# jantonguirao/nvImageCodec

Measured on AMD Instinct MI355X. Metric: images/sec, batched 1920x1080 4:2:0 baseline JPEG decode to interleaved RGB u8, higher is better.
Workload: dtype int32

## Files before the change

### include/hipjpeg.h

```cpp
#ifndef HIPJPEG_H_
#define HIPJPEG_H_

#include <stddef.h>
#include <stdint.h>

#ifdef __cplusplus
extern "C" {
#endif

#define HIPJPEG_API __attribute__((visibility("default")))

typedef enum {
    HIPJPEG_STATUS_SUCCESS = 0,
    HIPJPEG_STATUS_INVALID_ARGUMENT = 1,
    HIPJPEG_STATUS_BAD_JPEG = 2,
    HIPJPEG_STATUS_UNSUPPORTED = 3,
    HIPJPEG_STATUS_TRUNCATED = 4,
    HIPJPEG_STATUS_CORRUPT = 5,
    HIPJPEG_STATUS_ALLOC_FAILED = 6,
    HIPJPEG_STATUS_HIP_ERROR = 7,
    HIPJPEG_STATUS_NO_DEVICE = 8,
    HIPJPEG_STATUS_BUFFER_TOO_SMALL = 9,
    HIPJPEG_STATUS_INTERNAL_ERROR = 10
} hipjpegStatus_t;

typedef enum {
    HIPJPEG_OUTPUT_RGBI = 0,
    HIPJPEG_OUTPUT_BGRI = 1,
    HIPJPEG_OUTPUT_RGB_PLANAR = 2,
    HIPJPEG_OUTPUT_BGR_PLANAR = 3,
    HIPJPEG_OUTPUT_Y = 4,
    HIPJPEG_OUTPUT_YUV_PLANAR = 5
} hipjpegOutputFormat_t;

typedef enum {
    HIPJPEG_CSS_444 = 0,
    HIPJPEG_CSS_422 = 1,
    HIPJPEG_CSS_420 = 2,
    HIPJPEG_CSS_440 = 3,
    HIPJPEG_CSS_411 = 4,
    HIPJPEG_CSS_410 = 5,
    HIPJPEG_CSS_GRAY = 6,
    HIPJPEG_CSS_410V = 7,
    HIPJPEG_CSS_UNKNOWN = -1
} hipjpegChromaSubsampling_t;

#define HIPJPEG_FLAG_FANCY_UPSAMPLING 1u
#define HIPJPEG_FLAG_GPU_HUFFMAN 2u
#define HIPJPEG_FLAG_FAST_IDCT 4u
#define HIPJPEG_FLAG_GPU_PROGRESSIVE_INTERVALS 16u

typedef struct {
    int32_t width, height, num_components;
    int32_t sof_marker;
    int32_t color_model;
    int32_t subsampling;
    int32_t restart_interval, num_scans;
    int32_t h[4], v[4];
    int32_t blocks_w[4], blocks_h[4];
    int32_t samp_w[4], samp_h[4];
    uint64_t coef_bytes;
} hipjpegImageInfo_t;

typedef struct {
    void* plane[3];
    uint32_t pitch[3];
} hipjpegOutput_t;

typedef struct {
    int32_t x0, y0, x1, y1;
    int32_t orientation;
} hipjpegTransform_t;

typedef struct hipjpegHandle* hipjpegHandle_t;

HIPJPEG_API const char* hipjpegStatusString(hipjpegStatus_t status);
HIPJPEG_API int hipjpegVersion(void);
HIPJPEG_API hipjpegStatus_t hipjpegTestSetFault(const char* site, int countdown);
HIPJPEG_API int hipjpegTestDoubleReports(void);
HIPJPEG_API int32_t hipjpegTestHostFallbacks(hipjpegHandle_t handle);
HIPJPEG_API hipjpegStatus_t hipjpegTestKernelFlavours(hipjpegHandle_t handle, int32_t plane_units[1], int32_t luma_units[3]);
HIPJPEG_API int32_t hipjpegTestFusedUnits(hipjpegHandle_t handle);

HIPJPEG_API int32_t hipjpegTestScanChunkDrops(const uint8_t* data, size_t length, int scan_index, uint32_t* drops, int32_t capacity);
HIPJPEG_API int32_t hipjpegTestPairSteps(const uint8_t bits[16], const uint8_t* vals, int32_t nvals, uint32_t* steps);

HIPJPEG_API hipjpegStatus_t hipjpegTestSetScratchFill(int byte);

HIPJPEG_API hipjpegStatus_t hipjpegGetImageInfo(const uint8_t* data, size_t length, hipjpegImageInfo_t* info);

HIPJPEG_API hipjpegStatus_t hipjpegEntropyDecodeHost(const uint8_t* data, size_t length, int16_t* coef, size_t coef_capacity_bytes,
                                                     uint64_t comp_offsets[4], uint16_t qtables[256]);

HIPJPEG_API hipjpegStatus_t hipjpegEntropyDecodeHostSparse(const uint8_t* data, size_t length, uint8_t* stream, size_t capacity_bytes, size_t* stream_bytes,
                                                           uint64_t table_offsets[4]);

HIPJPEG_API hipjpegStatus_t hipjpegEntropyDecodeGpuAlgorithmHost(const uint8_t* data, size_t length, int16_t* coef,
                                                                 size_t coef_capacity_bytes, uint64_t comp_offsets[4],
                                                                 int32_t* sync_passes);

HIPJPEG_API hipjpegStatus_t hipjpegEntropyDecodeGpuIntervalAlgorithmHost(const uint8_t* data, size_t length, int16_t* coef,
                                                                         size_t coef_capacity_bytes, uint64_t comp_offsets[4]);

HIPJPEG_API hipjpegStatus_t hipjpegCreate(hipjpegHandle_t* handle, int device_id, int num_host_threads);
HIPJPEG_API hipjpegStatus_t hipjpegDestroy(hipjpegHandle_t handle);

typedef struct {
    int (*device_malloc)(void* ctx, void** ptr, size_t size, void* stream);
    int (*device_free)(void* ctx, void* ptr, size_t size, void* stream);
    void* device_ctx;
    int (*pinned_malloc)(void* ctx, void** ptr, size_t size, void* stream);
    int (*pinned_free)(void* ctx, void* ptr, size_t size, void* stream);
    void* pinned_ctx;
} hipjpegAllocators_t;
HIPJPEG_API hipjpegStatus_t hipjpegSetAllocators(hipjpegHandle_t handle, const hipjpegAllocators_t* allocators);

HIPJPEG_API hipjpegStatus_t hipjpegDecodeBatch(hipjpegHandle_t handle, const uint8_t* const* data, const size_t* lengths, int batch_size,
                                               const hipjpegOutput_t* outputs, hipjpegOutputFormat_t format, unsigned flags,
                                               hipjpegStatus_t* statuses, void* stream);

HIPJPEG_API hipjpegStatus_t hipjpegDecodeBatchSetTransforms(hipjpegHandle_t handle, const hipjpegTransform_t* transforms, int batch_size);

HIPJPEG_API hipjpegStatus_t hipjpegGetScaledImageSize(int32_t width, int32_t height, int32_t scale_denom, int32_t* scaled_width,
                                                      int32_t* scaled_height);
HIPJPEG_API hipjpegStatus_t hipjpegDecodeBatchSetScales(hipjpegHandle_t handle, const int32_t* scale_denoms, int batch_size);

HIPJPEG_API hipjpegStatus_t hipjpegDecodeBatchHost(hipjpegHandle_t handle, const uint8_t* const* data, const size_t* lengths, int batch_size,
                                                   const hipjpegOutput_t* outputs, hipjpegOutputFormat_t format, unsigned flags,
                                                   hipjpegStatus_t* statuses);
HIPJPEG_API hipjpegStatus_t hipjpegDecodeBatchTransfer(hipjpegHandle_t handle, void* stream);
HIPJPEG_API hipjpegStatus_t hipjpegDecodeBatchDevice(hipjpegHandle_t handle, void* stream);
HIPJPEG_API hipjpegStatus_t hipjpegDecodeBatchDeviceKernel(hipjpegHandle_t handle, int which, void* stream);
HIPJPEG_API hipjpegStatus_t hipjpegDecodeBatchSubmit(hipjpegHandle_t handle, const uint8_t* const* data, const size_t* lengths, int batch_size,
                                                     const hipjpegOutput_t* outputs, hipjpegOutputFormat_t format, unsigned flags, void* stream);
HIPJPEG_API hipjpegStatus_t hipjpegDecodeBatchWait(hipjpegHandle_t handle, hipjpegStatus_t* statuses, int batch_size);
HIPJPEG_API int32_t hipjpegDecodeBatchZeroCopyImages(hipjpegHandle_t handle);
HIPJPEG_API int32_t hipjpegDecodeBatchIntervalImages(hipjpegHandle_t handle);
HIPJPEG_API int32_t hipjpegDecodeBatchIntervalTakeovers(hipjpegHandle_t handle);
HIPJPEG_API hipjpegStatus_t hipjpegDecodeBatchTransferStats(hipjpegHandle_t handle, uint64_t* h2d_bytes, int32_t* sparse_images);

HIPJPEG_API hipjpegStatus_t hipjpegSetHybridHuffmanThreshold(hipjpegHandle_t handle, uint64_t pixels);

HIPJPEG_API hipjpegStatus_t hipjpegSetPipelineDepth(hipjpegHandle_t handle, int depth);
HIPJPEG_API hipjpegStatus_t hipjpegDecodeBatchGetStatuses(hipjpegHandle_t handle, hipjpegStatus_t* statuses, int batch_size);
HIPJPEG_API hipjpegStatus_t hipjpegDecodeBatchEntropyStats(hipjpegHandle_t handle, int32_t* gpu_images, int32_t* sync_launches,
                                                           uint64_t* stream_bytes);
HIPJPEG_API hipjpegStatus_t hipjpegDecodeBatchStats(hipjpegHandle_t handle, int32_t num_units[3], uint64_t* coef_bytes,
                                                    uint64_t* output_bytes);

typedef struct {
    const void* plane[3];
    uint32_t pitch[3];
    int32_t width, height;
} hipjpegEncodeInput_t;

typedef struct {
    int32_t quality;
    int32_t subsampling;
    int32_t input_format;
    int32_t restart_interval;
    int32_t optimized_huffman;
    int32_t progressive;
} hipjpegEncodeParams_t;
#define HIPJPEG_FLAG_GPU_RESTART_INTERVALS 8u
#define HIPJPEG_FLAG_GPU_PROGRESSIVE_RESTART 32u

HIPJPEG_API hipjpegStatus_t hipjpegEncodeBatchDevice(hipjpegHandle_t handle, const hipjpegEncodeInput_t* inputs,
                                                     const hipjpegEncodeParams_t* params, int batch_size, hipjpegStatus_t* statuses, void* stream);
// ... 134 lines not shown
```

### nvimagecodec_amd/csrc/decoder_core.cpp

```cpp
#include "decoder_core.h"
#include "host_copy.h"

#include <hip/hip_runtime_api.h>

#include <algorithm>
#include <cstdio>
#include <cstdlib>
#include <cstring>
#include <numeric>

#include "coefficients_core.h"
#include "decode_kernels.h"
#include "diagnostics.h"
#include "entropy_decode.h"
#include "gpu_huffman_host.h"
#include "progressive_gpu_host.h"
#include "transcode_core.h"

namespace hipjpeg {

namespace {
int out_planes(OutFormat fmt) { return (fmt == kOutInterleavedRGB || fmt == kOutInterleavedBGR || fmt == kOutY) ? 1 : 3; }
int out_bpp(OutFormat fmt) { return (fmt == kOutInterleavedRGB || fmt == kOutInterleavedBGR) ? 3 : 1; }

// ... 197 lines not shown
                                  hipjpegOutputFormat_t format, unsigned flags, hipjpegStatus_t* statuses,
                                  const hipjpegOutputFormat_t* formats, ForkJoinPool* pool, const hipjpegTransform_t* transforms,
                                  const int32_t* scale_denoms)
{
    pool_ = pool;
    coef_only_ = false;
    tensor_source_ = false;
    PlanArgs a{data, lengths, outputs, format, flags, formats, transforms, nullptr};
    a.scales = scale_denoms;
    return plan_attempts(a, n, statuses);
}

hipjpegStatus_t DecodeBatch::plan_tensors(const hipjpegCoefficientInfo_t* infos, const hipjpegCoefficientPlanes_t* planes, int n,
                                          const hipjpegOutput_t* outputs, hipjpegOutputFormat_t format, unsigned flags, hipjpegStatus_t* statuses,
                                          ForkJoinPool* pool, const hipjpegTransform_t* transforms)
{
    if (n > 0 && (!infos || !planes)) return HIPJPEG_STATUS_INVALID_ARGUMENT;
    pool_ = pool;
    coef_only_ = false;
    tensor_source_ = true;
    tensor_planes_ = planes;
    PlanArgs a{nullptr, nullptr, outputs, format, flags & ~HIPJPEG_FLAG_GPU_HUFFMAN, nullptr, transforms, nullptr};
    a.infos = infos;
    a.tensors = planes;
    return plan_attempts(a, n, statuses);
}

hipjpegStatus_t DecodeBatch::plan_coefficients(const uint8_t* const* data, const size_t* lengths, int n, unsigned flags, hipjpegStatus_t* statuses,
                                               ForkJoinPool* pool, const hipjpegTranscodeParams_t* params, bool any_frame)
{
    pool_ = pool;
    coef_only_ = true;
    tensor_source_ = false;
    return plan_attempts(PlanArgs{data, lengths, nullptr, HIPJPEG_OUTPUT_RGBI, flags & (HIPJPEG_FLAG_GPU_HUFFMAN | HIPJPEG_FLAG_GPU_PROGRESSIVE_INTERVALS), nullptr, nullptr, nullptr, params, any_frame}, n,
                         statuses);
}

hipjpegStatus_t DecodeBatch::plan_attempts(const PlanArgs& a, int n, hipjpegStatus_t* statuses)
{
    std::vector<char> give_up((size_t)std::max(n, 0), 0);
    PlanArgs args = a;
    args.give_up = give_up.data();
    for (int attempt = 0;; attempt++) {
        const hipjpegStatus_t st = plan_once(args, n, statuses);
        if (st != HIPJPEG_STATUS_ALLOC_FAILED || attempt >= 16) return st;
        int worst = -1;
        size_t worst_bytes = 0;
        for (int i = 0; i < n; i++) {
            if (images_[i].status != HIPJPEG_STATUS_SUCCESS) continue;
            const size_t b = images_[i].frame.total_blocks() * 128 + (size_t)images_[i].frame.width * images_[i].frame.height;
            if (b >= worst_bytes) {
                worst_bytes = b;
                worst = i;
            }
        }
        if (worst < 0) return st;
        give_up[worst] = 1;
    }
}

hipjpegStatus_t DecodeBatch::plan_once(const PlanArgs& a, int n, hipjpegStatus_t* statuses)
{
    if (n < 0 || (n > 0 && (((!a.data || !a.lengths) && !a.infos) || (!a.outputs && !coef_only_)))) return HIPJPEG_STATUS_INVALID_ARGUMENT;
    if ((int)a.format < 0 || (int)a.format > (int)HIPJPEG_OUTPUT_YUV_PLANAR) return HIPJPEG_STATUS_INVALID_ARGUMENT;
    ScopedRange range("hipjpeg plan (parse headers, lay out staging)");
    fault_point("plan");
    finalized_ = false;
    host_drops_missing_.store(false, std::memory_order_relaxed);
    images_.resize((size_t)n);
    desc_.resize((size_t)n);
    fast_idct_ = (a.flags & HIPJPEG_FLAG_FAST_IDCT) != 0;
    entropy_done_ = false;
    entropy_pending_ = false;
    huff_images_.clear();
    huff_to_image_.clear();
    seq_gpu_images_ = 0;
    prog_images_.clear();
    prog_to_image_.clear();
    prog_walk_images_ = 0;
    interval_takeover_images_ = 0;
    host_fallback_images_ = 0;
    xform_desc_.clear();
    prog_slot_words_ = 0;
    max_huff_units_ = max_pool_words_ = 0;
    coef_bytes_ = output_bytes_ = 0;
    if (pool_ && n > 1)
        pool_->parallel_for(n, [&](int i, int) { prepare(i, a); });
    else
        for (int i = 0; i < n; i++) prepare(i, a);
    demote_progressive_lds();
    for (int tail = 0; tail < 2; tail++) {
        for (int i = 0; i < n; i++) {
            PlannedImage& im = images_[i];
            if (im.status != HIPJPEG_STATUS_SUCCESS || !im.gpu_prog || (int)im.gpu_prog_intervals != tail) continue;
            im.prog_index = (int)prog_to_image_.size();
            prog_to_image_.push_back(i);
        }
        if (tail == 0) prog_walk_images_ = prog_to_image_.size();
    }
    Sizing s(n);
    for (int i = 0; i < n; i++) size_image(i, s);
    layout(s);
    const hipjpegStatus_t st = reserve(s);
    if (st != HIPJPEG_STATUS_SUCCESS) return st;
    bind_pointers(s);
    h2d_used_ = staging_.h2d_bytes;
    if (statuses)
        for (int i = 0; i < n; i++) statuses[i] = images_[i].status;
    return HIPJPEG_STATUS_SUCCESS;
}

void DecodeBatch::prepare(int i, const PlanArgs& a)
{
    PlannedImage& im = images_[i];
    im = PlannedImage();
    desc_[i] = DecodeImage();
    im.data = a.infos ? nullptr : a.data[i];
    im.size = a.infos ? 0 : a.lengths[i];
    if (a.formats && ((int)a.formats[i] < 0 || (int)a.formats[i] > (int)HIPJPEG_OUTPUT_YUV_PLANAR)) {
        im.status = HIPJPEG_STATUS_INVALID_ARGUMENT;
        return;
    }
    const OutFormat fmt = (OutFormat)(a.formats ? a.formats[i] : a.format);
    bool fancy = (a.flags & HIPJPEG_FLAG_FANCY_UPSAMPLING) != 0;
    const FrameInfo& f = im.frame;
    const int denom = a.scales ? a.scales[i] : 1;
    if (denom != 1 && denom != 2 && denom != 4 && denom != 8) {
        im.status = HIPJPEG_STATUS_INVALID_ARGUMENT;
        return;
    }
    im.scale_k = 8 / denom;
    if (a.infos)
        im.status = coefficient_frame(a.infos[i], a.tensors[i], &im.frame);
    else
        im.status = a.data[i] ? status_from_parse(parse_jpeg(a.data[i], a.lengths[i], &im.frame)) : HIPJPEG_STATUS_INVALID_ARGUMENT;
    if (im.status == HIPJPEG_STATUS_SUCCESS && ((uint64_t)f.width * (uint64_t)f.height * (uint64_t)f.ncomp >= max_image_samples() || a.give_up[i]))
        im.status = HIPJPEG_STATUS_ALLOC_FAILED;
    if (coef_only_) {
        TranscodePicture pic;
        im.variant = -4;
        const bool grayscale = a.transcode && (a.transcode[i].orientation & HIPJPEG_TRANSCODE_GRAYSCALE) != 0;
        if (im.status == HIPJPEG_STATUS_SUCCESS && !a.any_frame) im.status = transcode_picture(f, grayscale, &pic);
    } else {
        im.pic_w = f.width;
        im.pic_h = f.height;
        if (im.status == HIPJPEG_STATUS_SUCCESS && im.scale_k != 8) {
            im.variant = -5;
            im.pic_w = scaled_extent(f.width, im.scale_k);
            im.pic_h = scaled_extent(f.height, im.scale_k);
            fancy = fancy && im.scale_k > 1;
            if (!choose_scaled(f, fmt, im.scale_k, im.scaled_size)) im.status = HIPJPEG_STATUS_UNSUPPORTED;
        } else if (im.status == HIPJPEG_STATUS_SUCCESS && !choose_variant(f, fmt, fancy, &im.variant))
            im.status = HIPJPEG_STATUS_UNSUPPORTED;
        for (int p = 0; im.status == HIPJPEG_STATUS_SUCCESS && p < (fmt == kOutPlanarYUV ? f.ncomp : out_planes(fmt)); p++)
            if (!a.outputs[i].plane[p]) im.status = HIPJPEG_STATUS_INVALID_ARGUMENT;
        if (im.status == HIPJPEG_STATUS_SUCCESS && a.transforms) im.status = normalise_transform(im, a.transforms[i], fmt);
        if (im.status == HIPJPEG_STATUS_SUCCESS && !pitch_ok(i, a.outputs[i], fmt)) im.status = HIPJPEG_STATUS_INVALID_ARGUMENT;
    }
    const bool want_gpu_entropy = (a.flags & HIPJPEG_FLAG_GPU_HUFFMAN) != 0;
    const bool big_enough = (uint64_t)f.width * (uint64_t)f.height > gpu_entropy_min_pixels_ || gpu_entropy_min_pixels_ == 0;
    if (im.status == HIPJPEG_STATUS_SUCCESS && want_gpu_entropy && big_enough && gpu_entropy_eligible(f)) {
        im.gpu_entropy = true;
        for (const ScanHeader& sc : f.scans) im.pool_words = std::max(im.pool_words, gpu_pool_words(sc));
        im.fused_layout = f.scans.size() == 1;
        for (int c = 0; c < f.scans[0].ncomp; c++) im.fused_layout = im.fused_layout && f.scans[0].comp_index[c] == c;
        static const bool zero_copy = getenv("HIPJPEG_NO_ZERO_COPY") == nullptr;
        if (zero_copy) {
// ... 126 lines not shown
    }
    for (int c = 0; c < f.ncomp && im.variant == -5; c++) {
        const Component& k = f.comp[c];
        DecodeComponent& dc = d.comp[c];
        const size_t sz = (size_t)im.scaled_size[c];
        dc.plane_pitch = (uint32_t)align_up((size_t)k.blocks_w * sz + 16, 16);
        s.plane_off[(size_t)i * 4 + c] = s.planes.take(align_up((size_t)dc.plane_pitch * k.blocks_h * sz + 16, 256));
        s.units += ((size_t)k.blocks_w * k.blocks_h + kBlocksPerUnit - 1) / kBlocksPerUnit;
    }
    if (im.variant == -5) s.units += ((size_t)im.pic_h + kScaledRowsPerUnit - 1) / kScaledRowsPerUnit;
    for (int c = 0; c < f.ncomp && im.variant != -5; c++) {
        const Component& k = f.comp[c];
        const Route route = component_route(im.variant, fmt, c);
        if (route == kRoutePlane) {
            DecodeComponent& dc = d.comp[c];
            dc.plane_pitch = (uint32_t)align_up((size_t)k.blocks_w * 8 + 16, 16);
            s.plane_off[(size_t)i * 4 + c] = s.planes.take(align_up((size_t)dc.plane_pitch * k.blocks_h * 8 + 16, 256));
        }
        if (route != kRouteNone) s.units += ((size_t)k.blocks_w * k.blocks_h + kBlocksPerUnit - 1) / kBlocksPerUnit;
        if (c == 0 && im.variant >= 0) s.units += (size_t)((k.blocks_w + kLumaTileW - 1) / kLumaTileW) * (size_t)((k.blocks_h + kLumaTileH - 1) / kLumaTileH);
    }
    if (im.variant == -1 || im.variant == -3) s.units += (size_t)f.height;
    coef_bytes_ += f.total_blocks() * 128;
    if (tensor_source_)
        for (int c = 0; c < f.ncomp; c++) s.tensor_units += ((size_t)f.comp[c].blocks_w * f.comp[c].blocks_h + kRelayoutBlocksPerUnit - 1) / kRelayoutBlocksPerUnit;
    if (fmt == kOutPlanarYUV)
        for (int c = 0; c < f.ncomp; c++) output_bytes_ += (uint64_t)f.comp[c].samp_w * f.comp[c].samp_h;
    else
        output_bytes_ += (uint64_t)im.pic_w * im.pic_h * (fmt == kOutY ? 1 : 3);
    if (!im.gpu_entropy) return;
    if (im.gpu_prog) im.tables_offset = s.pools.take(align_up(im.pool_words * 2, 64), 1);
    if (!im.gpu_prog)
        for (size_t sidx = 0; sidx < f.scans.size(); sidx++) {
            const ScanHeader& sc = f.scans[sidx];
            const size_t blocks = (size_t)scan_mcus_x(f, sc) * scan_mcus_y(f, sc) * scan_blocks_per_mcu(f, sc);
            im.seq[sidx].dc_diff_offset = s.blocks.take(((blocks + 31) & ~(size_t)31) * 2, 1);
        }
    for (int c = 0; c < f.ncomp; c++) {
        const size_t nblk = (size_t)f.comp[c].blocks_w * f.comp[c].blocks_h;
        im.dc_plane_offset[c] = s.blocks.take(((nblk + 31) & ~(size_t)31) * 2, 1);
        if (im.gpu_prog) s.prog_units += (nblk + 255) / 256;
    }
    if (im.gpu_prog) {
        im.prog_huff_first = (uint32_t)s.prog_scans;
        s.prog_scans += f.scans.size();
        for (size_t sidx = 0; sidx < f.scans.size(); sidx++) {
            const ScanHeader& sc = f.scans[sidx];
            s.scan(sc, &im.prog_raw_offset[sidx], &im.prog_stream_offset[sidx], &im.prog_first_chunk[sidx]);
            if (sc.ss != 0) {
                const int cc = sc.comp_index[0];
                const size_t nb = (size_t)((f.comp[cc].samp_w + 7) / 8) * (size_t)((f.comp[cc].samp_h + 7) / 8);
                im.prog_pos_offset[sidx] = s.prog_pos.take(((nb + 63) & ~(size_t)63) * 4, 1);
                prog_slot_words_ = std::max<unsigned>(prog_slot_words_, (unsigned)prog_table_words(sc.ac[sc.ta[0]]));
            } else if (sc.ah == 0) {
                for (int k = 0; k < sc.ncomp; k++)
                    prog_slot_words_ = std::max<unsigned>(prog_slot_words_, (unsigned)prog_table_words(sc.dc[sc.td[k]]));
            }
        }
        if (im.gpu_prog_intervals) {
            int ac_scans[4] = {0, 0, 0, 0};
            for (size_t sidx = 0; sidx < f.scans.size(); sidx++) {
                const ScanHeader& sc = f.scans[sidx];
                const size_t count = sc.rst_after.size() + 1;
                im.prog_start_offset[sidx] = s.boundaries.take(align_up(sc.rst_after.size() * 4, 64), 1);
                if (sc.ss == 0 || ac_scans[sc.comp_index[0]]++ == 0) s.prog_iv_units += (count + kProgIntervalLanes - 1) / kProgIntervalLanes;
            }
            for (int c = 0; c < f.ncomp; c++)
                if (ac_scans[c] > 1)
                    im.prog_hist_offset[c] = s.prog_pos.take((size_t)((f.comp[c].samp_w + 7) / 8) * (size_t)((f.comp[c].samp_h + 7) / 8) * 8, 8);
        }
        return;
    }
    static_assert(sizeof(im.seq) / sizeof(im.seq[0]) == (size_t)kMaxSeqScans, "one SeqScan per scan gpu_entropy_eligible() admits");
    im.huff_index = (int)huff_to_image_.size();
    im.huff_count = (int)f.scans.size();
    seq_gpu_images_++;
    for (size_t sidx = 0; sidx < f.scans.size(); sidx++) {
        const ScanHeader& sc = f.scans[sidx];
        PlannedImage::SeqScan& q = im.seq[sidx];
        huff_to_image_.push_back(i);
        const size_t nsub = (s.scan(sc, &q.raw_offset, &q.stream_offset, &q.first_chunk) * 8 + kSubseqBits - 1) / kSubseqBits;
        const size_t mcus = (size_t)scan_mcus_x(f, sc) * scan_mcus_y(f, sc);
        s.subseq += nsub;
        max_huff_units_ += std::max<size_t>((nsub + kHuffOwn - 1) / kHuffOwn, 1);
        q.pool_words = gpu_pool_words(sc);
        q.tables_offset = s.pools.take(align_up(q.pool_words * 2, 64), 1);
        max_pool_words_ = std::max(max_pool_words_, q.pool_words);
        s.huff_wunits += (mcus + kHuffMcusPerWg - 1) / kHuffMcusPerWg + 1;
        q.num_boundaries = (uint32_t)sc.rst_after.size();
        q.boundary_offset = s.boundaries.take(sc.restart_interval ? align_up(((size_t)q.num_boundaries + nsub + 1) * 4, 64) : 0, 1);
        q.block_pos_offset = s.block_pos.take(((mcus * scan_blocks_per_mcu(f, sc) + 63) & ~(size_t)63) * 4, 1);
    }
}

void DecodeBatch::layout(const Sizing& s)
{
    const size_t ng = huff_to_image_.size(), chunks = s.chunks.end;
    StagingLayout& L = staging_;
    Carve c;
    L.desc = c.take(sizeof(DecodeImage) * images_.size());
    L.units = c.take(sizeof(WorkUnit) * s.units);
    L.huff_desc = c.take(sizeof(HuffImage) * (ng + s.prog_scans));
    L.huff_units = c.take(sizeof(HuffUnit) * max_huff_units_);
    L.huff_wunits = c.take(sizeof(HuffUnit) * s.huff_wunits);
    L.huff_dc_units = c.take(sizeof(HuffUnit) * ng * 4);
    L.huff_chunk_units = c.take(sizeof(HuffUnit) * chunks);
    L.huff_drops = c.take(sizeof(uint32_t) * chunks);
    L.xform_desc = c.take(sizeof(TransformImage) * xform_desc_.size());
    L.xform_units = c.take(sizeof(WorkUnit) * s.xform_units);
    L.prog_desc = c.take(sizeof(ProgImage) * prog_to_image_.size());
    L.prog_units = c.take(sizeof(HuffUnit) * s.prog_units);
    L.prog_iv_desc = c.take(sizeof(ProgIntervalImage) * (prog_to_image_.size() - prog_walk_images_));
    L.prog_iv_units = c.take(sizeof(HuffUnit) * s.prog_iv_units);
    L.tensor_planes = c.take(tensor_source_ ? sizeof(CoefPlane) * 4 * images_.size() : 0);
    L.tensor_units = c.take(sizeof(RelayoutUnit) * s.tensor_units);
    L.tables = c.take(s.pools.end);
    L.boundaries = c.take(s.boundaries.end);
    L.streams = c.take(s.raw.end);
    L.coef = c.take(0);
    static const bool sparse_enabled = getenv("HIPJPEG_DENSE_STAGING") == nullptr;
    sparse_mode_ = sparse_enabled && !coef_only_ && !tensor_source_;
    host_coef_used_.store(0);
    for (int pass = 0; pass < 2; pass++) {
        if (pass == 1) {
            L.h2d_bytes = c.end;
            L.gpu_coef_begin = c.take(0);
        }
        for (PlannedImage& im : images_) {
            if (im.status != HIPJPEG_STATUS_SUCCESS || (int)(im.gpu_entropy || tensor_source_) != pass) continue;
            if (pass == 0 && sparse_mode_) c.end += 256;
            for (int k = 0; k < im.frame.ncomp; k++) im.coef_offset[k] = c.take((size_t)im.frame.comp[k].blocks_w * im.frame.comp[k].blocks_h * 128, 1);
            if (!im.gpu_entropy) continue;
            if (im.gpu_prog) {
                im.tables_offset += L.tables;
                for (size_t sidx = 0; sidx < im.frame.scans.size(); sidx++) im.prog_raw_offset[sidx] += L.streams;
                for (size_t sidx = 0; sidx < im.frame.scans.size() && im.gpu_prog_intervals; sidx++) im.prog_start_offset[sidx] += L.boundaries;
            } else {
                for (int sidx = 0; sidx < im.huff_count; sidx++) {
                    im.seq[sidx].raw_offset += L.streams;
                    im.seq[sidx].boundary_offset += L.boundaries;
                    im.seq[sidx].tables_offset += L.tables;
                }
            }
        }
    }
    L.total = c.end;
    total_subseq_ = s.subseq;
    Carve w;
    w.take(total_subseq_ * 8);
    scratch_.first_block = w.take(total_subseq_ * 4);
    scratch_.changed = w.take(256);
    scratch_.incoming = w.take(max_huff_units_ * 8);
    scratch_.tail = w.take(max_huff_units_ * (kTailTaskBytes + 4));
    scratch_.dc_diff = w.take(s.blocks.end);
    scratch_.block_pos = w.take(s.block_pos.end);
    scratch_.records = w.take(total_subseq_ * kRecShorts * 2);
    scratch_.walkers = w.take(max_huff_units_ * 4);
    scratch_.verdicts = w.take(verdict_bytes());
    scratch_.drops = w.take(chunks * 4);
    scratch_.prog_pos = w.take(s.prog_pos.end);
    scratch_.group_sums = w.take(s.huff_wunits * 16);
    scratch_.streams = w.take(s.streams.end);
    scratch_.total = w.end;
}

hipjpegStatus_t DecodeBatch::reserve(const Sizing& s)
{
    if (hipSetDevice(device_id_) != hipSuccess) return HIPJPEG_STATUS_NO_DEVICE;
    if (in_flight_) {
        if (hipEventSynchronize((hipEvent_t)done_event_) != hipSuccess) return HIPJPEG_STATUS_HIP_ERROR;
        in_flight_ = false;
    }
    hipjpegStatus_t st;
    if ((st = pinned_.reserve(staging_.h2d_bytes + 256 + verdict_bytes())) != HIPJPEG_STATUS_SUCCESS) return st;
    if ((st = device_.reserve(staging_.total + 256)) != HIPJPEG_STATUS_SUCCESS) return st;
    if ((st = planes_.reserve(s.planes.end + 256)) != HIPJPEG_STATUS_SUCCESS) return st;
    if (!huff_to_image_.empty() || s.prog_scans) return work_.reserve(scratch_.total + 256);
    return HIPJPEG_STATUS_SUCCESS;
}

void DecodeBatch::bind_pointers(const Sizing& s)
{
    huff_images_.assign(huff_to_image_.size() + s.prog_scans, HuffImage());
    prog_images_.assign(prog_to_image_.size(), ProgImage());
    prog_iv_images_.assign(prog_to_image_.size() - prog_walk_images_, ProgIntervalImage());
    size_t k = 0;
// ... 157 lines not shown
    build_entropy_units();
    build_tensor_units();
    h2d_used_ = sparse_mode_ ? std::min(staging_.h2d_bytes, align_up(staging_.coef + host_coef_used_.load(), 256)) : staging_.h2d_bytes;
    stage_tables();
    finalized_ = true;
}

void DecodeBatch::build_pixel_units()
{
    for (UnitList* l : {&plane_units_, &fused_plane_units_, &generic_units_, &cmyk_units_, &xform_units_, &reduced_units_, &scaled_color_units_}) l->units.clear();
    for (auto* lists : {&luma_units_, &fused_luma_units_})
        for (auto& row : *lists)
            for (UnitList& l : row) l.units.clear();
    for (size_t i = 0; i < images_.size(); i++) {
        const PlannedImage& im = images_[i];
        if (im.status != HIPJPEG_STATUS_SUCCESS) continue;
        const FrameInfo& f = im.frame;
        DecodeImage& d = desc_[i];
        if (sparse_mode_ && !im.gpu_entropy) {
            size_t blocks_before = 0;
            for (int c = 0; c < f.ncomp; c++) {
                DecodeComponent& dc = d.comp[c];
                if (im.sparse) {
                    dc.coef = at<const int16_t>(device_, im.host_coef_offset);
                    dc.block_off = at<const uint32_t>(device_, im.host_coef_offset) + blocks_before;
                    blocks_before += (size_t)f.comp[c].blocks_w * f.comp[c].blocks_h;
                } else {
                    dc.coef = at<const int16_t>(device_, im.coef_offset[c]);
                    dc.block_off = nullptr;
                }
                dc.dc = dc.coef;
                dc.dc_stride = 64;
            }
        }
        const OutFormat fmt = (OutFormat)d.out_format;
        const bool fused = fused_ && im.gpu_entropy && !im.gpu_prog;
        d.huff_index = fused ? (uint32_t)im.huff_index : 0u;
        for (int c = 0; c < f.ncomp && im.variant == -5; c++) {
            const uint32_t nblk = (uint32_t)f.comp[c].blocks_w * f.comp[c].blocks_h;
            std::vector<WorkUnit>& list = (im.scaled_size[c] == 8 ? plane_units_ : reduced_units_).units;
            for (uint32_t b = 0; b < nblk; b += kBlocksPerUnit) list.push_back(WorkUnit{(uint32_t)i, b, (uint32_t)c, (uint32_t)kToPlane});
        }
        for (int y = 0; y < im.pic_h && im.variant == -5; y += kScaledRowsPerUnit) scaled_color_units_.units.push_back(WorkUnit{(uint32_t)i, (uint32_t)y, 0u, 0u});
        for (int c = 0; c < f.ncomp && im.variant != -5; c++) {
            const Route route = component_route(im.variant, fmt, c);
            if (route == kRouteNone) continue;
            const uint32_t nblk = (uint32_t)f.comp[c].blocks_w * f.comp[c].blocks_h;
            const uint32_t mode = route == kRouteOutput ? (uint32_t)(kToOutput | (c << 8)) : (uint32_t)kToPlane;
            for (uint32_t b = 0; b < nblk; b += kBlocksPerUnit) (fused ? fused_plane_units_ : plane_units_).units.push_back(WorkUnit{(uint32_t)i, b, (uint32_t)c, mode});
        }
        if (im.variant >= 0) {
            uint32_t real_rows = (uint32_t)(f.height + 7) / 8, first_row = 0, first_col = 0, end_col = (uint32_t)f.comp[0].blocks_w;
            if (im.has_transform) {
                first_row = (uint32_t)im.transform.y0 / 8 / kLumaTileH * kLumaTileH;
                real_rows = std::min(real_rows, (uint32_t)(im.transform.y1 + 7) / 8);
                first_col = (uint32_t)im.transform.x0 / 8 / kLumaTileW * kLumaTileW;
                end_col = std::min(end_col, (uint32_t)(im.transform.x1 + 7) / 8);
            }
            const bool everyday = im.variant != kVarGray && d.color_model == 1 && (d.flags & kFlagFancyUpsampling) &&
                                  (im.variant == kVar11 || im.variant == kVar12 || d.comp[1].samp_w > 2);
            const int layout = !everyday ? 0 : (fmt == kOutInterleavedRGB || fmt == kOutInterleavedBGR) ? 1 : (fmt == kOutPlanarRGB || fmt == kOutPlanarBGR) ? 2 : 0;
            std::vector<WorkUnit>& tiles = (fused ? fused_luma_units_ : luma_units_)[layout][im.variant].units;
            const uint32_t span = end_col - first_col, ragged = span % kLumaTileW;
            const uint32_t wide_end = (ragged != 0 && ragged <= kLumaTileW / 2) ? end_col - ragged : end_col;
            for (uint32_t by = first_row; by < real_rows; by += kLumaTileH)
                for (uint32_t bx = first_col; bx < wide_end; bx += kLumaTileW) tiles.push_back(WorkUnit{(uint32_t)i, bx, by, 0u});
            if (wide_end < end_col)
                for (uint32_t by = first_row; by < real_rows; by += 2 * kLumaTileH) tiles.push_back(WorkUnit{(uint32_t)i, wide_end, by, 1u});
        } else if (im.variant == -1) {
            for (int y = 0; y < f.height; y++) generic_units_.units.push_back(WorkUnit{(uint32_t)i, (uint32_t)y, 0u, 0u});
        } else if (im.variant == -3) {
            for (int y = 0; y < f.height; y++) cmyk_units_.units.push_back(WorkUnit{(uint32_t)i, (uint32_t)y, 0u, 0u});
        }
        if (im.has_transform) {
            const TransformImage& t = xform_desc_[im.xform_index];
            for (int oy = 0; oy < t.out_h; oy += kTransformRowsPerUnit) xform_units_.units.push_back(WorkUnit{(uint32_t)im.xform_index, (uint32_t)oy, 0u, 0u});
        }
    }
}

void DecodeBatch::build_entropy_units()
{
    for (std::vector<HuffUnit>* v : {&huff_units_, &huff_wunits_, &huff_chunk_units_, &huff_dc_units_, &prog_units_}) v->clear();
    uint32_t first_subseq = 0;
    stream_bytes_total_ = 0;
    huff_zero_.clear();
    for (size_t g = 0; g < huff_to_image_.size(); g++) {
        const PlannedImage& im = images_[huff_to_image_[g]];
        HuffImage& h = huff_images_[g];
        if (im.status != HIPJPEG_STATUS_SUCCESS) {
            h.num_subseq = 0;
            continue;
        }
        const int sidx = (int)g - im.huff_index;
        const ScanHeader& sc = im.frame.scans[sidx];
        const PlannedImage::SeqScan& q = im.seq[sidx];
        h.stream = work_.data() + scratch_.streams + q.stream_offset;
        h.raw = device_.data() + q.raw_offset;
        h.raw_src = im.input_pinned ? im.input_device_view + sc.data_begin : nullptr;
        if (h.restart_interval) {
            h.boundaries = at<const uint32_t>(device_, q.boundary_offset);
            h.sub_boundary = h.boundaries + h.num_boundaries;
        }
        h.raw_bytes = q.stream_bytes;
        h.first_chunk = q.first_chunk;
        for (uint32_t c = 0; c * (uint32_t)kDestuffChunk < q.stream_bytes; c++) huff_chunk_units_.push_back(HuffUnit{(uint32_t)g, c});
        h.pool = at<const uint16_t>(device_, q.tables_offset);
        h.dc_diff = at<int16_t>(work_, scratch_.dc_diff + q.dc_diff_offset);
        h.block_pos = at<uint32_t>(work_, scratch_.block_pos + q.block_pos_offset);
        for (uint32_t m = 0; m < h.mcus_x * h.mcus_y; m += kHuffMcusPerWg) huff_wunits_.push_back(HuffUnit{(uint32_t)g, m});
        for (int i = 0; i < sc.ncomp; i++) {
            const int c = sc.comp_index[i];
            const Component& fc = im.frame.comp[c];
            h.coef[i] = at<int16_t>(device_, im.coef_offset[c]);
            h.dc_plane[i] = at<int16_t>(work_, scratch_.dc_diff + im.dc_plane_offset[c]);
            const size_t bw = (size_t)fc.blocks_w, bh = (size_t)fc.blocks_h;
            if (sc.ncomp == 1 && (h.mcus_x < bw || h.mcus_y < bh)) {
                const size_t first = h.mcus_x < bw ? 0 : (size_t)h.mcus_y * bw, n = bw * bh - first;
                huff_zero_.push_back(ZeroFill{reinterpret_cast<uint8_t*>(h.coef[i] + first * 64), n * 128, 1, 0});
                huff_zero_.push_back(ZeroFill{reinterpret_cast<uint8_t*>(h.dc_plane[i] + first), n * 2, 1, 0});
            }
        }
        h.first_subseq = first_subseq;
        first_subseq += h.num_subseq;
        for (uint32_t j = 0; j == 0 || j < h.num_subseq; j += kHuffOwn) huff_units_.push_back(HuffUnit{(uint32_t)g, j});
        if (h.restart_interval)
            for (uint32_t i = 0; i < h.ncomp; i++) huff_dc_units_.push_back(HuffUnit{(uint32_t)g, i});
        stream_bytes_total_ += q.stream_bytes;
    }
    merge_zero_fills();
    total_subseq_ = first_subseq;
    for (size_t q = 0; q < prog_images_.size(); q++) {
        const PlannedImage& im = images_[prog_to_image_[q]];
        ProgImage& pi = prog_images_[q];
        if (im.status != HIPJPEG_STATUS_SUCCESS) {
            pi.num_scans = 0;
            pi.ncomp = 0;
            pi.dc_len = 0;
            memset(pi.chain_len, 0, sizeof pi.chain_len);
            continue;
        }
        const FrameInfo& f = im.frame;
        for (size_t sidx = 0; sidx < f.scans.size(); sidx++) {
            const size_t hidx = huff_to_image_.size() + im.prog_huff_first + sidx;
            HuffImage& h = huff_images_[hidx];
            h.stream = work_.data() + scratch_.streams + im.prog_stream_offset[sidx];
            h.raw = device_.data() + im.prog_raw_offset[sidx];
            ProgScan& ps = pi.scan[sidx];
            ps.stream = h.stream;
            ps.huff_image = (uint32_t)hidx;
            ps.block_pos = f.scans[sidx].ss != 0 ? at<uint32_t>(work_, scratch_.prog_pos + im.prog_pos_offset[sidx]) : nullptr;
            for (uint32_t c = 0; c * (uint32_t)kDestuffChunk < h.raw_bytes; c++) huff_chunk_units_.push_back(HuffUnit{(uint32_t)hidx, c});
        }
        pi.pool = at<const uint16_t>(device_, im.tables_offset);
        for (int c = 0; c < f.ncomp; c++) {
            pi.coef[c] = at<int16_t>(device_, im.coef_offset[c]);
            pi.dc_plane[c] = at<int16_t>(work_, scratch_.dc_diff + im.dc_plane_offset[c]);
            const uint32_t nblk = (uint32_t)f.comp[c].blocks_w * f.comp[c].blocks_h;
            for (uint32_t b = 0; b < nblk; b += 256) prog_units_.push_back(HuffUnit{(uint32_t)q, ((uint32_t)c << 28) | b});
        }
        stream_bytes_total_ += im.stream_bytes;
    }
    prog_iv_units_.clear();
    prog_iv_dc_first_.clear();
    uint32_t dc_scans = 0;
    for (size_t q = prog_walk_images_; q < prog_images_.size(); q++) {
        const PlannedImage& im = images_[prog_to_image_[q]];
        if (im.status != HIPJPEG_STATUS_SUCCESS) continue;
        const uint32_t rel = (uint32_t)(q - prog_walk_images_);
        ProgIntervalImage& iv = prog_iv_images_[rel];
        for (size_t sidx = 0; sidx < im.frame.scans.size(); sidx++) iv.scan[sidx].first_start = (uint32_t)((im.prog_start_offset[sidx] - staging_.boundaries) / 4);
        for (int c = 0; c < im.frame.ncomp; c++) {
            iv.hist[c] = prog_images_[q].chain_len[c] > 1 ? at<unsigned long long>(work_, scratch_.prog_pos + im.prog_hist_offset[c]) : nullptr;
            for (uint32_t first = 0; prog_images_[q].chain_len[c] > 0 && first < iv.ac_count[c]; first += kProgIntervalLanes)
                prog_iv_units_.push_back(HuffUnit{rel, ((uint32_t)c << 28) | first});
        }
        dc_scans = std::max(dc_scans, prog_images_[q].dc_len);
    }
    for (uint32_t d = 0; d < dc_scans; d++) {
        prog_iv_dc_first_.push_back(prog_iv_units_.size());
        for (size_t q = prog_walk_images_; q < prog_images_.size(); q++) {
            const ProgImage& pi = prog_images_[q];
            if (pi.dc_len <= d) continue;
            const uint32_t count = prog_iv_images_[q - prog_walk_images_].scan[pi.dc_chain[d]].count;
            for (uint32_t first = 0; first < count; first += kProgIntervalLanes) prog_iv_units_.push_back(HuffUnit{(uint32_t)(q - prog_walk_images_), first});
        }
    }
    prog_iv_dc_first_.push_back(prog_iv_units_.size());
}

void DecodeBatch::merge_zero_fills()
{
    std::vector<ZeroFill> in, out;
    in.swap(huff_zero_);
    for (int series = 0; series < 2; series++) {
        for (size_t a = (size_t)series; a < in.size();) {
            ZeroFill z = in[a];
            size_t b = a + 2;
            if (b < in.size() && in[b].bytes == z.bytes && in[b].ptr > z.ptr && (size_t)(in[b].ptr - z.ptr) >= z.bytes) {
                z.pitch = (size_t)(in[b].ptr - z.ptr);
                while (b < in.size() && in[b].bytes == z.bytes && in[b].ptr == z.ptr + z.count * z.pitch) {
                    z.count++;
                    b += 2;
                }
            }
            out.push_back(z);
            a += 2 * z.count;
        }
    }
    huff_zero_.swap(out);
}

static void deal_rows_to_xcds(std::vector<WorkUnit>& v)
{
    if (v.size() < 64) return;
    constexpr size_t kXcds = 8;
    std::vector<WorkUnit> queue[kXcds], rest, out;
    out.reserve(v.size());
    auto flush = [&]() {
        size_t taken[kXcds] = {0};
        for (bool any = true; any;) {
            any = false;
            for (size_t q = 0; q < kXcds; q++)
                if (taken[q] < queue[q].size()) {
                    out.push_back(queue[q][taken[q]++]);
                    any = true;
                }
        }
        out.insert(out.end(), rest.begin(), rest.end());
        for (auto& q : queue) q.clear();
        rest.clear();
    };
    size_t row = 0;
    for (size_t a = 0; a < v.size();) {
        size_t b = a + 1;
        while (b < v.size() && v[b].image == v[a].image && v[b].comp == v[a].comp && v[b].mode == v[a].mode) b++;
        if (a > 0 && v[a].image != v[a - 1].image) {
            flush();
            row = 0;
        }
        if (v[a].mode != 0) {
            rest.insert(rest.end(), v.begin() + (long)a, v.begin() + (long)b);
        } else {
            std::vector<WorkUnit>& q = queue[row++ % kXcds];
            q.insert(q.end(), v.begin() + (long)a, v.begin() + (long)b);
        }
        a = b;
    }
    flush();
    v.swap(out);
}

void DecodeBatch::stage_tables()
{
    auto stage = [&](UnitList& list, Carve& where) {
        list.offset = where.take(list.units.size() * sizeof(WorkUnit), 1);
        copy_table(pinned_, list.offset, list.units);
    };
    copy_table(pinned_, staging_.desc, desc_);
    Carve units{staging_.units};
    stage(plane_units_, units);
    for (auto& lists : luma_units_)
        for (UnitList& l : lists) {
            deal_rows_to_xcds(l.units);
            stage(l, units);
        }
    stage(fused_plane_units_, units);
    for (auto& lists : fused_luma_units_)
        for (UnitList& l : lists) stage(l, units);
    stage(generic_units_, units);
    stage(cmyk_units_, units);
    stage(reduced_units_, units);
    stage(scaled_color_units_, units);
    Carve xform{staging_.xform_units};
    stage(xform_units_, xform);
    copy_table(pinned_, staging_.xform_desc, xform_desc_);
    copy_table(pinned_, staging_.tensor_planes, tensor_table_);
    copy_table(pinned_, staging_.tensor_units, tensor_units_);
    copy_table(pinned_, staging_.prog_desc, prog_images_);
    copy_table(pinned_, staging_.prog_units, prog_units_);
    copy_table(pinned_, staging_.prog_iv_desc, prog_iv_images_);
    copy_table(pinned_, staging_.prog_iv_units, prog_iv_units_);
    copy_table(pinned_, staging_.huff_desc, huff_images_);
    copy_table(pinned_, staging_.huff_units, huff_units_);
    copy_table(pinned_, staging_.huff_wunits, huff_wunits_);
    copy_table(pinned_, staging_.huff_dc_units, huff_dc_units_);
    copy_table(pinned_, staging_.huff_chunk_units, huff_chunk_units_);
}

hipjpegStatus_t DecodeBatch::transfer(void* stream, bool kernels_on_other_stream)
{
    if (!finalized_) return HIPJPEG_STATUS_INVALID_ARGUMENT;
    ScopedRange range("hipjpeg transfer to device");
    fault_point("transfer");
    entropy_done_ = false;
    pixels_launched_ = false;
    if (h2d_used_ == 0) return HIPJPEG_STATUS_SUCCESS;
    zero_copy_images_ = 0;
    for (const PlannedImage& im : images_) zero_copy_images_ += (im.status == HIPJPEG_STATUS_SUCCESS && im.gpu_entropy && !im.gpu_prog && im.input_pinned) ? 1 : 0;
    hipError_t e = hipSuccess;
    if (zero_copy_images_ == 0) {
        e = hipMemcpyAsync(device_.data(), pinned_.data(), h2d_used_, hipMemcpyHostToDevice, (hipStream_t)stream);
    } else {
        hipStream_t s = (hipStream_t)stream;
        const size_t rb = std::min(staging_.streams, h2d_used_), re = std::min(staging_.coef, h2d_used_);
        if (rb > 0) e = hipMemcpyAsync(device_.data(), pinned_.data(), rb, hipMemcpyHostToDevice, s);
        if (e == hipSuccess && re > rb) e = hipMemsetAsync(device_.data() + rb, 0x01, re - rb, s);
        if (e == hipSuccess && h2d_used_ > re) e = hipMemcpyAsync(device_.data() + re, pinned_.data() + re, h2d_used_ - re, hipMemcpyHostToDevice, s);
        for (const PlannedImage& im : images_) {
            if (e != hipSuccess) break;
            if (im.status != HIPJPEG_STATUS_SUCCESS || !im.gpu_entropy) continue;
            if (im.gpu_prog) {
                for (size_t sidx = 0; sidx < im.frame.scans.size() && e == hipSuccess; sidx++) {
                    const ScanHeader& sc = im.frame.scans[sidx];
                    const size_t len = sc.data_end - sc.data_begin;
                    if (len) e = hipMemcpyAsync(device_.data() + im.prog_raw_offset[sidx], pinned_.data() + im.prog_raw_offset[sidx], align_up(len, 16) + 16, hipMemcpyHostToDevice, s);
                }
                continue;
            }
            for (int sidx = 0; sidx < im.huff_count && e == hipSuccess && !im.input_pinned; sidx++) {
                const PlannedImage::SeqScan& q = im.seq[sidx];
                e = hipMemcpyAsync(device_.data() + q.raw_offset, pinned_.data() + q.raw_offset, align_up((size_t)q.stream_bytes, 16) + 16, hipMemcpyHostToDevice, s);
            }
        }
        if (e == hipSuccess && launch_gather_raw(at<const HuffImage>(device_, staging_.huff_desc), at<const HuffUnit>(device_, staging_.huff_chunk_units),
                                                 (int)huff_chunk_units_.size(), stream) != 0) e = hipErrorLaunchFailure;
    }
    if (e == hipSuccess && kernels_on_other_stream) {
        if (!ensure_event(&copied_event_)) return HIPJPEG_STATUS_HIP_ERROR;
        e = hipEventRecord((hipEvent_t)copied_event_, (hipStream_t)stream);
        copy_pending_ = true;
    }
    return e == hipSuccess ? HIPJPEG_STATUS_SUCCESS : HIPJPEG_STATUS_HIP_ERROR;
}

hipjpegStatus_t DecodeBatch::enqueue_gpu_entropy(void* stream)
{
    hipStream_t s = (hipStream_t)stream;
    entropy_done_ = true;
    if (huff_units_.empty() && prog_units_.empty()) return HIPJPEG_STATUS_SUCCESS;
    EntropyLaunch L = entropy_launch_args();
    if (huff_chunk_units_.empty() && hipMemsetAsync(L.changed, 0, 256, s) != hipSuccess) return HIPJPEG_STATUS_HIP_ERROR;
    for (const ZeroFill& z : huff_zero_)
        if ((z.count == 1 ? hipMemsetAsync(z.ptr, 0, z.bytes, s) : hipMemset2DAsync(z.ptr, z.pitch, 0, z.bytes, z.count, s)) != hipSuccess)
            return HIPJPEG_STATUS_HIP_ERROR;
    static const bool force_device_count = getenv("HIPJPEG_DEVICE_DESTUFF_COUNT") != nullptr;
    const bool device_count = force_device_count || host_drops_missing_.load(std::memory_order_relaxed);
    if (launch_destuff(L.dimg, at<const HuffUnit>(device_, staging_.huff_chunk_units), (int)huff_chunk_units_.size(),
                       device_count ? at<uint32_t>(work_, scratch_.drops) : at<uint32_t>(device_, staging_.huff_drops),
                       device_count, L.changed, stream) != 0)
        return HIPJPEG_STATUS_HIP_ERROR;
    if (!prog_units_.empty()) {
        const hipjpegStatus_t ps = enqueue_progressive(stream);
        if (ps != HIPJPEG_STATUS_SUCCESS) return ps;
    }
    if (huff_units_.empty()) {
        entropy_pending_ = true;
        return HIPJPEG_STATUS_SUCCESS;
    }
    static const int tail_after = getenv("HIPJPEG_TAIL_AFTER") ? atoi(getenv("HIPJPEG_TAIL_AFTER")) : 2;
    uint16_t* tail_tasks = at<uint16_t>(work_, scratch_.tail);
    uint32_t* tail_count = at<uint32_t>(work_, scratch_.tail + (size_t)max_huff_units_ * kTailTaskBytes);
    if (launch_huff_sync(L.dimg, L.dunits, L.nunits, L.states, L.incoming, L.changed, 1, tail_after > 0 ? tail_after : 1 << 20,
                         tail_after > 0 ? tail_tasks : nullptr, tail_after > 0 ? tail_count : nullptr, L.records, L.pool_bytes, stream) != 0)
        return HIPJPEG_STATUS_HIP_ERROR;
    if (launch_huff_sync(L.dimg, L.dunits, L.nunits, L.states, L.incoming, L.changed, 0, 1 << 20, nullptr, nullptr, L.records, L.pool_bytes, stream, 1) != 0)
        return HIPJPEG_STATUS_HIP_ERROR;
    if (!entropy_write_passes(L, stream)) return HIPJPEG_STATUS_HIP_ERROR;
    if (L.verdicts_out != L.host_changed && hipMemcpyAsync(L.host_changed, L.verdicts_out, verdict_bytes(), hipMemcpyDeviceToHost, s) != hipSuccess)
        return HIPJPEG_STATUS_HIP_ERROR;
    if (fused_ && hipMemcpyAsync(L.himg, L.dimg, sizeof(HuffImage) * huff_images_.size(), hipMemcpyDeviceToHost, s) != hipSuccess) return HIPJPEG_STATUS_HIP_ERROR;
    entropy_pending_ = true;
    return HIPJPEG_STATUS_SUCCESS;
}

hipjpegStatus_t DecodeBatch::enqueue_progressive(void* stream)
{
    ProgImage* dprog = at<ProgImage>(device_, staging_.prog_desc);
    const HuffImage* dimg = at<const HuffImage>(device_, staging_.huff_desc);
    const unsigned slot = (unsigned)align_up(std::max<unsigned>(prog_slot_words_, 256u), 64);
    unsigned dc_slots = 1, ac_waves = 0, rings = 0;
    for (size_t q = 0; q < prog_walk_images_; q++) {
        const ProgImage& pi = prog_images_[q];
        unsigned scans = 0, handovers = 0;
        for (int c = 0; c < 4; c++) {
            scans += pi.chain_len[c];
            handovers += pi.chain_len[c] > 0 ? pi.chain_len[c] - 1 : 0;
        }
        ac_waves = std::max(ac_waves, scans);
        rings = std::max(rings, handovers);
        for (uint32_t k = 0; k < pi.num_scans; k++)
            if (pi.scan[k].ss == 0 && pi.scan[k].ah == 0) dc_slots = std::max<unsigned>(dc_slots, pi.scan[k].ncomp);
    }
    static const bool debug_stats = getenv("HIPJPEG_DEBUG_TIMING") != nullptr;
    if (debug_stats)
        fprintf(stderr, "[hipjpeg] progressive walk: %zu images, %u + 1 waves per workgroup, %u table slots of %u entries, %u rings; interval kernels: %zu images\n",
                prog_walk_images_, ac_waves, dc_slots + ac_waves, slot, rings, prog_images_.size() - prog_walk_images_);
    if (launch_prog_walk(dprog, dimg, (int)prog_walk_images_, slot, dc_slots, ac_waves, rings, stream) != 0) return HIPJPEG_STATUS_HIP_ERROR;
    if (!prog_iv_units_.empty()) {
        ProgImage* tail = dprog + prog_walk_images_;
        const ProgIntervalImage* ivs = at<const ProgIntervalImage>(device_, staging_.prog_iv_desc);
        const uint32_t* starts = at<const uint32_t>(device_, staging_.boundaries);
        const HuffUnit* units = at<const HuffUnit>(device_, staging_.prog_iv_units);
        if (launch_prog_interval_ac(tail, ivs, dimg, starts, units, (int)prog_iv_dc_first_[0], slot, stream) != 0) return HIPJPEG_STATUS_HIP_ERROR;
        for (size_t d = 0; d + 1 < prog_iv_dc_first_.size(); d++)
            if (launch_prog_interval_dc(tail, ivs, dimg, starts, units + prog_iv_dc_first_[d], (int)(prog_iv_dc_first_[d + 1] - prog_iv_dc_first_[d]), (unsigned)d,
                                        slot, stream) != 0)
                return HIPJPEG_STATUS_HIP_ERROR;
    }
    if (launch_prog_replay(dprog, dimg, at<const HuffUnit>(device_, staging_.prog_units), (int)prog_units_.size(), slot, stream) != 0)
        return HIPJPEG_STATUS_HIP_ERROR;
    if (hipMemcpyAsync(pinned_.data() + staging_.prog_desc, dprog, sizeof(ProgImage) * prog_images_.size(), hipMemcpyDeviceToHost,
                       (hipStream_t)stream) != hipSuccess)
        return HIPJPEG_STATUS_HIP_ERROR;
    return HIPJPEG_STATUS_SUCCESS;
}

DecodeBatch::EntropyLaunch DecodeBatch::entropy_launch_args()
{
    EntropyLaunch L;
    L.dimg = at<HuffImage>(device_, staging_.huff_desc);
    L.dunits = at<const HuffUnit>(device_, staging_.huff_units);
    L.dwunits = at<const HuffUnit>(device_, staging_.huff_wunits);
    L.ddc = at<const HuffUnit>(device_, staging_.huff_dc_units);
    L.states = at<unsigned long long>(work_, 0);
    L.first_block = at<uint32_t>(work_, scratch_.first_block);
    static const bool full_position_pass = getenv("HIPJPEG_POSITION_PASS") != nullptr && atoi(getenv("HIPJPEG_POSITION_PASS")) != 0;
    L.records = at<uint16_t>(work_, scratch_.records);
    L.use_records = !full_position_pass && total_subseq_ * kRecShorts * 2 < (1ull << 32) ? L.records : nullptr;
    L.walkers = at<uint32_t>(work_, scratch_.walkers);
    L.group_sums = at<int32_t>(work_, scratch_.group_sums);
    L.changed = at<unsigned int>(work_, scratch_.changed);
    L.incoming = at<unsigned long long>(work_, scratch_.incoming);
    L.pool_bytes = (unsigned)align_up(max_pool_words_ * 2, 256);
    L.nunits = (int)huff_units_.size();
    L.host_changed = at<unsigned int>(pinned_, staging_.h2d_bytes);
    L.verdicts = L.host_changed + kHuffVerdictCounters;
    L.verdicts_out = pinned_.custom() ? at<unsigned int>(work_, scratch_.verdicts) : L.host_changed;
    L.himg = at<HuffImage>(pinned_, staging_.huff_desc);
    return L;
}

bool DecodeBatch::entropy_write_passes(const EntropyLaunch& L, void* stream)
{
    return launch_huff_write(L.dimg, L.dunits, L.nunits, L.dwunits, (int)huff_wunits_.size(), L.states, L.first_block, L.use_records, L.walkers, L.group_sums, L.pool_bytes,
                             stream, fused_) == 0 &&
           launch_huff_dc(L.dimg, L.ddc, (int)huff_dc_units_.size(), L.dwunits, (int)huff_wunits_.size(), L.group_sums, L.changed, L.verdicts_out, stream) == 0;
}

hipjpegStatus_t DecodeBatch::wait_done()
{
    if (!in_flight_) return HIPJPEG_STATUS_SUCCESS;
    return hipEventSynchronize((hipEvent_t)done_event_) == hipSuccess ? HIPJPEG_STATUS_SUCCESS : HIPJPEG_STATUS_HIP_ERROR;
}

hipjpegStatus_t DecodeBatch::resolve(void* stream)
{
    if (!entropy_pending_) return HIPJPEG_STATUS_SUCCESS;
    ScopedRange range("hipjpeg resolve (GPU entropy verdicts)");
    fault_point("resolve");
    hipStream_t s = (hipStream_t)stream;
    if (in_flight_ ? hipEventSynchronize((hipEvent_t)done_event_) != hipSuccess : hipStreamSynchronize(s) != hipSuccess) return HIPJPEG_STATUS_HIP_ERROR;
    entropy_pending_ = false;
    const EntropyLaunch L = entropy_launch_args();
    const size_t himg_bytes = sizeof(HuffImage) * huff_images_.size();
    bool redo_pixels = false;
    last_sync_launches_ = 2;
    static const bool debug_stats = getenv("HIPJPEG_DEBUG_TIMING") != nullptr;
    if (debug_stats)
        fprintf(stderr, "[hipjpeg] entropy: %d workgroups, launch 1 rounds avg %.2f max %u, tail rounds avg %.2f max %u; launch 2: %u rounds in total, max %u, %u boundary changes\n",
                L.nunits, (double)L.host_changed[2] / L.nunits, L.host_changed[3], (double)L.host_changed[6] / L.nunits, L.host_changed[7], L.host_changed[4],
                L.host_changed[5], L.host_changed[0]);
    bool converged = huff_units_.empty() || *L.host_changed == 0;
    constexpr int kExtraRippleLaunches = 4;
    uint32_t last_pass = 1;
    std::vector<char> unsettled(huff_images_.size(), 0);
    bool from_desc = fused_;
    if (!converged) {
        from_desc = true;
        for (int pass = 0; pass < kExtraRippleLaunches && !converged; pass++) {
            if (hipMemsetAsync(L.changed, 0, sizeof(unsigned int), s) != hipSuccess) return HIPJPEG_STATUS_HIP_ERROR;
            if (launch_huff_sync(L.dimg, L.dunits, L.nunits, L.states, L.incoming, L.changed, 0, 1 << 20, nullptr, nullptr, L.records, L.pool_bytes, stream, ++last_pass) != 0)
                return HIPJPEG_STATUS_HIP_ERROR;
            if (hipMemcpyAsync(L.host_changed, L.changed, sizeof(unsigned int), hipMemcpyDeviceToHost, s) != hipSuccess) return HIPJPEG_STATUS_HIP_ERROR;
            if (hipStreamSynchronize(s) != hipSuccess) return HIPJPEG_STATUS_HIP_ERROR;
            last_sync_launches_++;
            converged = *L.host_changed == 0;
        }
        if (hipMemcpyAsync(L.himg, L.dimg, himg_bytes, hipMemcpyDeviceToHost, s) != hipSuccess) return HIPJPEG_STATUS_HIP_ERROR;
        if (hipStreamSynchronize(s) != hipSuccess) return HIPJPEG_STATUS_HIP_ERROR;
        for (size_t g = 0; g < huff_to_image_.size(); g++) {
            unsettled[g] = L.himg[g].gave_up != 0 || (!converged && L.himg[g].moved_pass == last_pass);
            L.himg[g].status = 0;
        }
        if (hipMemcpyAsync(L.dimg, L.himg, himg_bytes, hipMemcpyHostToDevice, s) != hipSuccess) return HIPJPEG_STATUS_HIP_ERROR;
        if (!entropy_write_passes(L, stream)) return HIPJPEG_STATUS_HIP_ERROR;
        if (fused_ && pixels_launched_ && launch_pixel_kernels(stream, -1) != 0) return HIPJPEG_STATUS_HIP_ERROR;
        if (hipMemcpyAsync(L.himg, L.dimg, himg_bytes, hipMemcpyDeviceToHost, s) != hipSuccess) return HIPJPEG_STATUS_HIP_ERROR;
        if (hipStreamSynchronize(s) != hipSuccess) return HIPJPEG_STATUS_HIP_ERROR;
        redo_pixels = true;
    } else {
        for (size_t g = 0; g < huff_to_image_.size(); g++) unsettled[g] = from_desc ? L.himg[g].gave_up != 0 : huff_verdict_gave_up(L.verdicts[g]);
    }
    std::vector<int> takeover;
    for (size_t g = 0; g < huff_to_image_.size(); g++) {
        const int i = huff_to_image_[g];
        const bool flagged = from_desc ? L.himg[g].status != 0 : huff_verdict_status(L.verdicts[g]) != 0;
        if (images_[i].status == HIPJPEG_STATUS_SUCCESS && (flagged || unsettled[g]) && (takeover.empty() || takeover.back() != i))
            takeover.push_back(i);
    }
    host_fallback_images_ = (int)takeover.size();
    const ProgImage* hprog = at<const ProgImage>(pinned_, staging_.prog_desc);
    if (debug_stats && !prog_to_image_.empty()) print_progressive_timing(hprog);
    interval_takeover_images_ = 0;
    for (size_t q = 0; q < prog_to_image_.size(); q++)
        if (images_[prog_to_image_[q]].status == HIPJPEG_STATUS_SUCCESS && hprog[q].status != 0) {
            takeover.push_back(prog_to_image_[q]);
            interval_takeover_images_ += q >= prog_walk_images_ ? 1 : 0;
        }
    const hipjpegStatus_t st = take_over_on_host(takeover, &redo_pixels);
    if (st != HIPJPEG_STATUS_SUCCESS) return st;
    if (redo_pixels && pixels_launched_) {
        if (launch_pixel_kernels(stream, -1) != 0 || hipStreamSynchronize(s) != hipSuccess) return HIPJPEG_STATUS_HIP_ERROR;
    }
    return HIPJPEG_STATUS_SUCCESS;
}

void DecodeBatch::print_progressive_timing(const ProgImage* hprog) const
{
    const ProgImage& q0 = hprog[0];
    for (uint32_t k = 0; k < q0.num_scans; k++) {
        uint32_t lo = ~0u, hi = 0, cnt = 0;
        double sum = 0;
        for (size_t q = 0; q < prog_to_image_.size(); q++) {
            if (hprog[q].num_scans <= k) continue;
            const uint32_t t = hprog[q].scan[k].walk_ticks;
            lo = std::min(lo, t);
            hi = std::max(hi, t);
            sum += t;
            cnt++;
        }
        const uint32_t hw = q0.scan[k].pad_ticks[0];
        fprintf(stderr,
                "[hipjpeg] progressive image 0 scan %u (ss %u se %u ah %u al %u): walk %.3f ms, of which waiting for neighbours %.3f ms; se %u cu %u simd %u; "
                "all %u images: %.3f / %.3f / %.3f ms\n",
                k, q0.scan[k].ss, q0.scan[k].se, q0.scan[k].ah, q0.scan[k].al, q0.scan[k].walk_ticks * 1e-5, q0.scan[k].wait_ticks * 1e-5, (hw >> 13) & 7u,
                (hw >> 8) & 15u, (hw >> 4) & 3u, cnt, lo * 1e-5, cnt ? sum / cnt * 1e-5 : 0.0, hi * 1e-5);
    }
}

hipjpegStatus_t DecodeBatch::take_over_on_host(const std::vector<int>& takeover, bool* redo_pixels)
{
    constexpr size_t kHelping = 32;
    for (size_t first = 0; first < takeover.size(); first += kHelping) {
        const size_t count = std::min(kHelping, takeover.size() - first);
        std::vector<std::vector<int16_t>> coefs(count);
        std::vector<EntropyStatus> verdict(count, kEntropyOk);
        auto decode_one = [&](int j) {
            const PlannedImage& im = images_[takeover[first + j]];
            const FrameInfo& f = im.frame;
            coefs[j].assign(f.total_blocks() * 64, 0);
            int16_t* coef[4] = {nullptr, nullptr, nullptr, nullptr};
            size_t off = 0;
            for (int c = 0; c < f.ncomp; c++) {
                coef[c] = coefs[j].data() + off;
// ... 310 lines not shown
```

### nvimagecodec_amd/csrc/decoder_core.h

```cpp
#pragma once
#include <algorithm>
#include <atomic>
#include <cstddef>
#include <cstdint>
#include <vector>

#include "../../include/hipjpeg.h"
#include "coefficient_kernels.h"
#include "device_layout.h"
#include "decode_kernels.h"
#include "gpu_huffman.h"
#include "progressive_gpu.h"
#include "jpeg_syntax.h"
#include "staging.h"
#include "thread_pool.h"

namespace hipjpeg {

enum KernelVariant { kVarGray = 0, kVar11 = 1, kVar21 = 2, kVar22 = 3, kVar12 = 4, kNumLumaVariants = 5 };

struct UnitList {
    std::vector<WorkUnit> units;
    size_t offset = 0;
};
// ... 43 lines not shown
    uint32_t prog_first_chunk[kProgMaxScans] = {0};
    size_t prog_pos_offset[kProgMaxScans] = {0};
    bool gpu_prog_intervals = false;
    size_t prog_start_offset[kProgMaxScans] = {0};
    size_t prog_hist_offset[4] = {0, 0, 0, 0};
};

class DecodeBatch {
public:
    DecodeBatch(int device_id, const MemoryHooks* hooks);
    ~DecodeBatch();

    hipjpegStatus_t plan(const uint8_t* const* data, const size_t* lengths, int n, const hipjpegOutput_t* outputs,
                         hipjpegOutputFormat_t format, unsigned flags, hipjpegStatus_t* statuses,
                         const hipjpegOutputFormat_t* formats = nullptr, ForkJoinPool* pool = nullptr,
                         const hipjpegTransform_t* transforms = nullptr, const int32_t* scale_denoms = nullptr);
    hipjpegStatus_t plan_coefficients(const uint8_t* const* data, const size_t* lengths, int n, unsigned flags, hipjpegStatus_t* statuses,
                                      ForkJoinPool* pool, const hipjpegTranscodeParams_t* params = nullptr, bool any_frame = false);
    hipjpegStatus_t plan_tensors(const hipjpegCoefficientInfo_t* infos, const hipjpegCoefficientPlanes_t* planes, int n, const hipjpegOutput_t* outputs,
                                 hipjpegOutputFormat_t format, unsigned flags, hipjpegStatus_t* statuses, ForkJoinPool* pool,
                                 const hipjpegTransform_t* transforms = nullptr);
    hipjpegStatus_t import_tensors(void* stream);
    uint64_t imported_blocks() const { return imported_blocks_; }
    hipjpegStatus_t export_coefficients(const hipjpegCoefficientPlanes_t* planes, void* stream);
    uint64_t exported_blocks() const { return exported_blocks_; }
    const DecodeImage* device_descriptors() const { return at<const DecodeImage>(device_, staging_.desc); }
    void set_gpu_entropy_threshold(uint64_t pixels) { gpu_entropy_min_pixels_ = pixels; }
    void reject(int i, hipjpegStatus_t st)
    {
        if (i >= 0 && i < (int)images_.size() && images_[i].status == HIPJPEG_STATUS_SUCCESS) images_[i].status = st;
    }
    void output_size(int i, int* w, int* h) const;
    void entropy_stage(int i);
    void finalize(hipjpegStatus_t* statuses);
    hipjpegStatus_t transfer(void* stream, bool kernels_on_other_stream = false);
    hipjpegStatus_t launch(void* stream, int which = -1, void* entropy_stream = nullptr);
    hipjpegStatus_t resolve(void* stream);
    hipjpegStatus_t wait_done();
    void* last_stream() const { return last_stream_; }
    int gpu_entropy_images() const { return seq_gpu_images_ + (int)prog_to_image_.size(); }
    int last_sync_launches() const { return last_sync_launches_; }
    int host_fallback_images() const { return host_fallback_images_; }
    bool has_progressive() const { return !prog_to_image_.empty(); }
    int interval_images() const { return (int)(prog_to_image_.size() - prog_walk_images_); }
    int interval_takeover_images() const { return interval_takeover_images_; }
    uint64_t stream_bytes() const { return stream_bytes_total_; }
    int zero_copy_images() const { return zero_copy_images_; }
    uint64_t h2d_bytes() const { return h2d_used_; }
    int sparse_images() const { return (int)std::count_if(images_.begin(), images_.end(), [](const PlannedImage& im) { return im.sparse; }); }
    void flavour_units(int32_t* plane_units, int32_t luma_units[kNumLumaLayouts]) const { unit_counts(true, plane_units, luma_units); }
    int fused_units() const;

    int size() const { return (int)images_.size(); }
    const PlannedImage& image(int i) const { return images_[i]; }
    void stats(int32_t num_units[3], uint64_t* coef_bytes, uint64_t* output_bytes) const;

private:
    int device_id_;
    ForkJoinPool* pool_ = nullptr;
    uint64_t gpu_entropy_min_pixels_ = 0;

    struct PlanArgs;
    struct Sizing;
    hipjpegStatus_t plan_attempts(const PlanArgs& a, int n, hipjpegStatus_t* statuses);
    bool coef_only_ = false;
    bool tensor_source_ = false;
    const hipjpegCoefficientPlanes_t* tensor_planes_ = nullptr;
    std::vector<CoefPlane> tensor_table_;
    std::vector<RelayoutUnit> tensor_units_;
    void build_tensor_units();
    uint64_t imported_blocks_ = 0;
    hipjpegStatus_t plan_once(const PlanArgs& a, int n, hipjpegStatus_t* statuses);
    void prepare(int i, const PlanArgs& a);
    bool pitch_ok(int i, const hipjpegOutput_t& out, OutFormat fmt) const;
    void demote_progressive_lds();
    void size_image(int i, Sizing& s);
    void layout(const Sizing& s);
    hipjpegStatus_t reserve(const Sizing& s);
    void bind_pointers(const Sizing& s);
    Buffer pinned_, device_, planes_;
    Buffer export_pinned_, export_device_;
    uint64_t exported_blocks_ = 0;
    struct StagingLayout {
        size_t desc, units, huff_desc, huff_units, huff_wunits, huff_dc_units, huff_chunk_units, huff_drops, xform_desc, xform_units,
            prog_desc, prog_units, prog_iv_desc, prog_iv_units, tensor_planes, tensor_units, tables, boundaries, streams, coef, h2d_bytes, gpu_coef_begin, total;
    } staging_{};
    struct WorkLayout {
        size_t first_block, changed, incoming, tail, dc_diff, block_pos, records, walkers, verdicts, drops, prog_pos, group_sums, streams, total;
    } scratch_{};
    size_t verdict_bytes() const { return (kHuffVerdictCounters + huff_to_image_.size()) * sizeof(unsigned int); }
    Buffer work_;
    std::vector<PlannedImage> images_;
    std::vector<DecodeImage> desc_;
    bool fast_idct_ = false;
    uint64_t coef_bytes_ = 0, output_bytes_ = 0;
    bool sparse_mode_ = false;
    std::atomic<size_t> host_coef_used_{0};
    size_t h2d_used_ = 0;
    void stage_chunk_drops(const ScanHeader& sc, uint32_t first_chunk);
    void build_pixel_units();
    void build_entropy_units();
    void stage_tables();
    void merge_zero_fills();
    void unit_counts(bool plain, int32_t* plane, int32_t luma[kNumLumaLayouts]) const;
    UnitList plane_units_, luma_units_[kNumLumaLayouts][kNumLumaVariants], generic_units_, cmyk_units_, xform_units_;
    UnitList reduced_units_, scaled_color_units_;
    UnitList fused_plane_units_, fused_luma_units_[kNumLumaLayouts][kNumLumaVariants];
    bool fused_ = false;
    bool finalized_ = false;
    std::vector<TransformImage> xform_desc_;
    std::vector<HuffImage> huff_images_;
    std::vector<HuffUnit> huff_units_, huff_dc_units_;
    std::vector<int> huff_to_image_;
    int seq_gpu_images_ = 0;
    struct ZeroFill {
        uint8_t* ptr;
        size_t bytes, count, pitch;
    };
    std::vector<ZeroFill> huff_zero_;
    std::vector<HuffUnit> huff_wunits_;
    std::vector<HuffUnit> huff_chunk_units_;
    size_t total_subseq_ = 0, max_huff_units_ = 0, max_pool_words_ = 0;
    std::atomic<bool> host_drops_missing_{false};
    std::vector<ProgImage> prog_images_;
    std::vector<int> prog_to_image_;
    std::vector<HuffUnit> prog_units_;
    unsigned prog_slot_words_ = 0;
    size_t prog_walk_images_ = 0;
    std::vector<ProgIntervalImage> prog_iv_images_;
    std::vector<HuffUnit> prog_iv_units_;
    std::vector<size_t> prog_iv_dc_first_;
    uint64_t stream_bytes_total_ = 0;
    struct EntropyLaunch {
        HuffImage* dimg;
        const HuffUnit *dunits, *dwunits, *ddc;
        unsigned long long *states, *incoming;
        uint32_t* first_block;
        uint16_t* records;
        const uint16_t* use_records;
        uint32_t* walkers;
        int32_t* group_sums;
        unsigned int *changed, *host_changed;
        unsigned int* verdicts;
        unsigned int* verdicts_out;
        HuffImage* himg;
        unsigned pool_bytes;
        int nunits;
    };
    EntropyLaunch entropy_launch_args();
    bool entropy_write_passes(const EntropyLaunch& L, void* stream);
    hipjpegStatus_t enqueue_gpu_entropy(void* stream);
    hipjpegStatus_t enqueue_progressive(void* stream);
    int launch_pixel_kernels(void* stream, int which);
    int launch_taken_pixels(void* stream, int which);
    void print_progressive_timing(const ProgImage* hprog) const;
    hipjpegStatus_t take_over_on_host(const std::vector<int>& takeover, bool* redo_pixels);
    int zero_copy_images_ = 0;
    std::vector<int> host_taken_;
    void* taken_units_dev_ = nullptr;
    size_t taken_units_cap_ = 0;
    bool entropy_pending_ = false, pixels_launched_ = false, copy_pending_ = false, entropy_done_ = false;
    void* last_stream_ = nullptr;
    void* copied_event_ = nullptr;
    void* entropy_event_ = nullptr;
    void* done_event_ = nullptr;
    bool in_flight_ = false;
    int last_sync_launches_ = 0, host_fallback_images_ = 0, interval_takeover_images_ = 0;
};

hipjpegStatus_t status_from_parse(ParseStatus s);

}
```

### nvimagecodec_amd/csrc/gpu_huffman.h

```cpp
#pragma once
#include <cstdint>

#include "huffman_gpu_core.h"

namespace hipjpeg {

struct HuffUnit {
    uint32_t image;
    uint32_t first;
};

int launch_gather_raw(const HuffImage* images, const HuffUnit* chunk_units, int nchunks, void* stream);
int launch_destuff(HuffImage* images, const HuffUnit* chunk_units, int nchunks, uint32_t* drops, bool count_on_device, unsigned int* counters,
                   void* stream);

int launch_huff_sync(HuffImage* images, const HuffUnit* units, int nunits, unsigned long long* states, unsigned long long* incoming,
                     unsigned int* changed, int first_pass, int max_rounds, uint16_t* tail_tasks, uint32_t* tail_count, uint16_t* records,
                     unsigned pool_bytes, void* stream, unsigned pass_id = 0);
int launch_huff_write(HuffImage* images, const HuffUnit* sync_units, int nsync_units, const HuffUnit* block_units, int nblock_units,
                      const unsigned long long* states, uint32_t* first_block, const uint16_t* records, uint32_t* walkers,
                      int32_t* group_sums, unsigned pool_bytes, void* stream, bool dc_only = false);
constexpr int kHuffVerdictCounters = 8;
constexpr uint32_t huff_verdict(uint32_t status, uint32_t gave_up) { return (status & 0xFFu) | (gave_up ? 0x100u : 0u); }
constexpr uint32_t huff_verdict_status(uint32_t v) { return v & 0xFFu; }
constexpr bool huff_verdict_gave_up(uint32_t v) { return (v & 0x100u) != 0; }
int launch_huff_dc(const HuffImage* images, const HuffUnit* rst_units, int nrst_units, const HuffUnit* block_units, int nblock_units,
                   const int32_t* group_sums, const unsigned int* counters, unsigned int* verdicts, void* stream);

}
```

### nvimagecodec_amd/csrc/gpu_huffman.hip

```cpp
#include <hip/hip_runtime.h>

#include "gpu_huffman.h"
#include "huffman_gpu_core.h"
#include "kernel_common.h"

namespace hipjpeg {

namespace {

constexpr int kThreads = 256;

constexpr int kRowShift = kSubseqWords == 32 ? 5 : kSubseqWords == 16 ? 4 : kSubseqWords == 64 ? 6 : -1;
static_assert(kRowShift > 0, "subsequences of 512, 1024 or 2048 bits");

struct KSlot {
    int16_t* base;
    uint32_t stride_y, stride_x;
};

constexpr int kStagedExtra = 2;
constexpr int kRowWords = kSubseqWords + kStagedExtra;
static_assert(kSubseqWords % 4 == 0 && kStagedExtra == 2, "stage_rows: 16-byte groups and one 8-byte group per row");
__host__ __device__ constexpr int staged_lds_words(int rows) { return rows * kRowWords; }

struct WgShared {
    uint32_t stream[staged_lds_words(kSyncThreads)];
    unsigned long long end[kSyncThreads];
    uint32_t tsel[10];
    uint32_t queue[kSyncThreads];
    uint32_t wave_count[kSyncThreads / 64];
};

__device__ __forceinline__ uint32_t load_boundary(const uint32_t* boundaries, uint32_t n, uint32_t i)
{
    return i < n ? ((const HJ_GLOBAL uint32_t*)boundaries)[i] : 0xFFFFFFFFu;
}

struct LdsTables {
    uint32_t pool;
    const HJ_LDS uint32_t* tsel;
    static __device__ __forceinline__ uint32_t index1(uint32_t w) { return (w >> (31 - kHuffFastBits)) & ((2u << kHuffFastBits) - 2); }
    static __device__ __forceinline__ uint32_t index2(uint32_t w) { return (w >> 15) & ((2u << kHuffSubBits) - 2); }
    __device__ __forceinline__ uint32_t tables(int k) const { return tsel[k]; }
    __device__ __forceinline__ uint32_t lookup1(uint32_t t, uint32_t w) const { return *(const HJ_LDS uint16_t*)(uintptr_t)(pool + t + index1(w)); }
    __device__ __forceinline__ uint32_t lookup2(uint32_t e, uint32_t w) const
    {
        return *(const HJ_LDS uint16_t*)(uintptr_t)(pool + ((e & 0x1FFu) << 7) + index2(w));
    }
    __device__ __forceinline__ uint32_t lookup_pair(uint32_t t, uint32_t w) const
    {
        return *(const HJ_LDS uint16_t*)(uintptr_t)(pool + t + 2 * kPairOffset + index1(w));
    }
};

__device__ __forceinline__ StepTables make_step_tables(const HuffImage& im, uint32_t pool)
{
    const auto of = [&](uint32_t q) { return ((uint32_t)im.k[q].tdc * 2) | ((uint32_t)im.k[q].tac * 2 << 16); };
    TableClasses c = make_countdown_classes(im.blocks_per_mcu, of);
#pragma unroll
    for (int i = 0; i < 4; i++) {
        c.pair[i] = HJ_UNIFORM(c.pair[i]);
        asm("" : "+v"(c.pair[i]));
    }
    c.bit0 = HJ_UNIFORM(c.bit0);
    c.bit1 = HJ_UNIFORM(c.bit1);
    StepTables s = split_classes(c, 1u, pool);
#pragma unroll
    for (int i = 0; i < 4; i++) {
        asm("" : "+v"(s.dc[i]));
        asm("" : "+v"(s.ac[i]));
    }
    return s;
}

struct DevEnv : LdsTables {
    uint32_t stream_base;
    uint32_t word0;
    uint32_t row_addr;
    uint32_t row_word0;
    StepTables step;
    const uint32_t* boundaries;
    uint32_t num_boundaries;
    __device__ __forceinline__ uint32_t boundary(uint32_t i) const { return load_boundary(boundaries, num_boundaries, i); }
    static constexpr uint32_t kCursorStep = (uint32_t)kSyncThreads * 4u;
    __device__ __forceinline__ void set_row(int row)
    {
        row_addr = stream_base + ((uint32_t)row << 2);
        row_word0 = word0 + ((uint32_t)row << kRowShift);
    }
    __device__ __forceinline__ uint32_t cursor(uint32_t i) const { return row_addr + (i - row_word0) * kCursorStep; }
    __device__ __forceinline__ uint32_t fetch(uint32_t c) const { return *(const HJ_LDS uint32_t*)(uintptr_t)c; }
};

__device__ __forceinline__ uint32_t boundary0_of(const HuffImage& im, uint32_t subseq)
{
    return im.restart_interval ? ((const HJ_GLOBAL uint32_t*)im.sub_boundary)[subseq] : 0u;
}
struct SlotRecorder {
    HJ_GLOBAL char* records;
    uint32_t off;
    uint32_t bit0;
    __device__ __forceinline__ void operator()(uint32_t i, uint32_t pos) const
    {
        *(HJ_GLOBAL uint16_t*)(records + (off + 2 * min(i, (uint32_t)kRecSlots))) = (uint16_t)(pos - bit0);
    }
};
__device__ __forceinline__ SlotRecorder slot_recorder(uint16_t* records, const HuffImage& im, uint32_t j)
{
    SlotRecorder r;
    r.records = (HJ_GLOBAL char*)records;
    r.off = (im.first_subseq + j) * (uint32_t)(2 * kRecShorts);
    r.bit0 = j * kSubseqBits;
    return r;
}
__device__ __forceinline__ void put_mark(const SlotRecorder& r, uint32_t begin, uint32_t limit, uint32_t total_bits, uint32_t z0, const SubseqState& st)
{
    *(HJ_GLOBAL uint16_t*)(r.records + (r.off + 2 * kRecMark)) = (uint16_t)record_mark(begin, min(limit, total_bits), z0, st);
}

template <bool FOUR>
struct StepEnv : DevEnv {
    __device__ __forceinline__ explicit StepEnv(const DevEnv& e) : DevEnv(e) {}
    __device__ __forceinline__ void step_tables(uint32_t d, uint32_t* tdc, uint32_t* tac) const { select_halves<FOUR>(step, d, tdc, tac); }
    __device__ __forceinline__ uint32_t step_entry(uint32_t t, uint32_t w) const { return *(const HJ_LDS uint16_t*)(uintptr_t)(t + index1(w)); }
    __device__ __forceinline__ uint32_t step_pair(uint32_t t, uint32_t w) const
    {
        return *(const HJ_LDS uint16_t*)(uintptr_t)(t + 2 * kPairOffset + index1(w));
    }
    __device__ __forceinline__ uint32_t step_second(uint32_t e) const { return second_table_of(e, 7u, pool); }
};
__device__ __forceinline__ SubseqState sync_walk(bool rst, bool record, const HuffGeom& geom, const DevEnv& env, uint32_t begin, uint32_t limit, int z, int k,
                                                 uint32_t boundary0, const SlotRecorder& rec)
{
    const auto walk = [&](const auto& senv) {
        if (rst) return select_walk<true>(geom, senv, begin, limit, z, k, boundary0);
        return record ? select_walk<false>(geom, senv, begin, limit, z, k, 0, rec) : select_walk<false>(geom, senv, begin, limit, z, k);
    };
    if (env.step.bit1 == 0) return walk(StepEnv<false>(env));
    return walk(StepEnv<true>(env));
}

template <int ROWS>
__device__ __forceinline__ void stage_rows(uint32_t* lds_stream, const HuffImage& im, int first_row)
{
    const int t = threadIdx.x;
    const HJ_GLOBAL uint32_t* g = (const HJ_GLOBAL uint32_t*)im.stream;
    const int nwords = (int)im.stream_words;
    const int w0 = (first_row + t) * kSubseqWords;
    constexpr int kGroups = kSubseqWords / 4;
    u32x4 v[kGroups];
    typedef unsigned int u32x2 __attribute__((ext_vector_type(2)));
    u32x2 tail;
    {
        const int gd = w0 + kSubseqWords;
        const int gc = min(max(gd, 0), (nwords - 1) & ~1);
        const u32x2 x = *(const HJ_GLOBAL u32x2*)(g + gc);
        tail = (gd >= 0 && gd < nwords) ? x : u32x2{~0u, ~0u};
    }
#pragma unroll
    for (int i = 0; i < kGroups; i++) {
        const int gd = w0 + i * 4;
        const int gc = min(max(gd, 0), (nwords - 1) & ~3);
        const u32x4 x = *(const HJ_GLOBAL u32x4*)(g + gc);
        v[i] = (gd >= 0 && gd < nwords) ? x : u32x4{~0u, ~0u, ~0u, ~0u};
    }
    HJ_LDS uint32_t* dst = (HJ_LDS uint32_t*)lds_stream + t;
#pragma unroll
    for (int i = 0; i < kGroups; i++) {
        dst[(4 * i + 0) * ROWS] = __builtin_bswap32(v[i].x);
        dst[(4 * i + 1) * ROWS] = __builtin_bswap32(v[i].y);
        dst[(4 * i + 2) * ROWS] = __builtin_bswap32(v[i].z);
        dst[(4 * i + 3) * ROWS] = __builtin_bswap32(v[i].w);
    }
    dst[(kSubseqWords + 0) * ROWS] = __builtin_bswap32(tail.x);
    dst[(kSubseqWords + 1) * ROWS] = __builtin_bswap32(tail.y);
}

template <int THREADS>
__device__ __forceinline__ void stage_pool(HJ_LDS uint16_t* pool, const HuffImage& im)
{
    const HJ_GLOBAL u32x4* gp = (const HJ_GLOBAL u32x4*)im.pool;
    const uint32_t npool = im.pool_words >> 3;
    for (uint32_t i = threadIdx.x; i < npool; i += THREADS) {
        const u32x4 x = gp[i];
        HJ_LDS uint32_t* lp = reinterpret_cast<HJ_LDS uint32_t*>(pool) + i * 4;
        lp[0] = x.x;
        lp[1] = x.y;
        lp[2] = x.z;
        lp[3] = x.w;
    }
}

__device__ __forceinline__ void stage_constants(uint32_t* tsel, KSlot* kslot, uint32_t* zzw, const HuffImage& im, bool with_addresses)
{
    const int t = threadIdx.x;
    if (t < 10) {
        const HuffK hk = im.k[t];
        tsel[t] = ((uint32_t)hk.tdc * 2) | ((uint32_t)hk.tac * 2 << 16);
        if (with_addresses) {
            KSlot s;
            s.base = im.coef[hk.comp & 3] + (size_t)hk.blk0 * 64;
            s.stride_y = hk.stride_y;
            s.stride_x = hk.stride_x;
            kslot[t] = s;
        }
    }
    if (zzw && t >= 64 && t < 80) {
        constexpr uint8_t zz[64] = HJ_ZIGZAG_DEVICE_TABLE;
        const int i = (t - 64) * 4;
        zzw[t - 64] = ((uint32_t)zz[i] | ((uint32_t)zz[i + 1] << 8) | ((uint32_t)zz[i + 2] << 16) | ((uint32_t)zz[i + 3] << 24)) << 1;
    }
}

__device__ __forceinline__ DevEnv make_env(WgShared& sh, HJ_LDS uint16_t* pool, uint32_t first, const HuffGeom& geom, const HuffImage& im)
{
    DevEnv env;
    env.stream_base = (uint32_t)(uintptr_t)(HJ_LDS uint32_t*)sh.stream;
    env.word0 = (first - 1) * kSubseqWords;
    env.row_addr = env.stream_base;
    env.row_word0 = env.word0;
    env.pool = (uint32_t)(uintptr_t)pool;
    env.tsel = (const HJ_LDS uint32_t*)sh.tsel;
    env.step = make_step_tables(im, env.pool);
    env.boundaries = geom.boundaries;
    env.num_boundaries = geom.num_boundaries;
    return env;
}

__device__ __forceinline__ int compact_tasks(WgShared& sh, bool has, int value, int* task)
{
    const int t = threadIdx.x;
    const unsigned long long mask = __ballot(has);
    const int below = __popcll(mask & ((1ull << (t & 63)) - 1));
    if ((t & 63) == 0) sh.wave_count[t >> 6] = (uint32_t)__popcll(mask);
    __syncthreads();
    int base = 0, n = 0;
#pragma unroll
    for (int w = 0; w < kSyncThreads / 64; w++) {
        const int c = (int)sh.wave_count[w];
        if (w < (t >> 6)) base += c;
        n += c;
    }
    if (has) sh.queue[base + below] = (uint32_t)value;
    __syncthreads();
    *task = t < n ? (int)sh.queue[t] : -1;
    return n;
}

constexpr int kGatherGroups = 64;
__global__ __launch_bounds__(kThreads) void gather_raw_kernel(const HuffImage* __restrict__ images, const HuffUnit* __restrict__ units, int nunits)
{
    for (int ui = blockIdx.x; ui < nunits; ui += gridDim.x) {
        const HuffUnit u = units[ui];
        const HuffImage& im = images[u.image];
        const uint8_t* src = im.raw_src;
        if (!src) continue;
        const uint32_t begin = u.first * (uint32_t)kDestuffChunk;
        if (begin >= im.raw_bytes) continue;
        const uint32_t n = min((uint32_t)kDestuffChunk, im.raw_bytes - begin);
        const uint8_t* s = src + begin;
        uint8_t* d = const_cast<uint8_t*>(im.raw) + begin;
        typedef u32x4 __attribute__((aligned(1))) u32x4_unaligned;
        for (uint32_t i = threadIdx.x * 16u; i + 16u <= n; i += kThreads * 16u) *(HJ_GLOBAL u32x4*)(d + i) = *(const HJ_GLOBAL u32x4_unaligned*)(s + i);
        const uint32_t tail = n & ~15u;
        if (threadIdx.x < (n & 15u)) d[tail + threadIdx.x] = s[tail + threadIdx.x];
    }
}


__device__ __forceinline__ uint32_t zero_bytes(uint32_t v) { return ~(((v & 0x7F7F7F7Fu) + 0x7F7F7F7Fu) | v | 0x7F7F7F7Fu); }

__device__ __forceinline__ uint32_t stuffed_zero_mask(uint32_t x, uint32_t prev) { return zero_bytes(x | ~((x << 8) | prev)); }

__device__ __forceinline__ uint32_t marker_mask(uint32_t x, uint32_t prev, uint32_t next)
{
    const uint32_t ff_x = zero_bytes(~x);
    const uint32_t rst_x = zero_bytes((x & 0xF8F8F8F8u) ^ 0xD0D0D0D0u);
    const uint32_t ff_before = (ff_x << 8) | (prev == 0xFFu ? 0x80u : 0u);
    const uint32_t after = (x >> 8) | (next << 24);
    return (rst_x & ff_before) | (ff_x & zero_bytes((after & 0xF8F8F8F8u) ^ 0xD0D0D0D0u));
}

__device__ __forceinline__ uint32_t stuffed_mask(uint32_t x, uint32_t prev, uint32_t next, bool markers)
{
    const uint32_t d = stuffed_zero_mask(x, prev);
    return markers ? d | marker_mask(x, prev, next) : d;
}

__device__ __forceinline__ uint32_t lane_masks(const uint8_t* p, bool has_prev, bool markers, uint32_t m[16], uint32_t x[16])
{
    const uint4* q = reinterpret_cast<const uint4*>(p);
    uint32_t prev = has_prev ? p[-1] : 0u;
    uint32_t n = 0;
#pragma unroll
    for (int i = 0; i < 4; i++) {
        const uint4 v = q[i];
        x[4 * i + 0] = v.x;
        x[4 * i + 1] = v.y;
        x[4 * i + 2] = v.z;
        x[4 * i + 3] = v.w;
    }
    const uint32_t behind = p[64];
#pragma unroll
    for (int i = 0; i < 16; i++) {
        m[i] = stuffed_mask(x[i], prev, i < 15 ? (x[i < 15 ? i + 1 : 15] & 0xFFu) : behind, markers);
        prev = x[i] >> 24;
        n += __popc(m[i]);
    }
    return n;
}

__device__ __forceinline__ uint32_t wg_sum(uint32_t v, uint32_t* scratch )
{
    for (int off = 32; off > 0; off >>= 1) v += __shfl_xor(v, off);
    if ((threadIdx.x & 63) == 0) scratch[threadIdx.x >> 6] = v;
    __syncthreads();
    const uint32_t total = scratch[0] + scratch[1] + scratch[2] + scratch[3];
    __syncthreads();
    return total;
}

__global__ __launch_bounds__(kThreads) void destuff_count_kernel(const HuffImage* __restrict__ images, const HuffUnit* __restrict__ units,
                                                                 uint32_t* __restrict__ drops)
{
    __shared__ uint32_t scratch[4];
    const HuffUnit u = units[blockIdx.x];
// ... 87 lines not shown
        uint32_t prev = before_lane;
#pragma unroll
        for (uint32_t i = 0; i < 16; i++) {
            d[i] = stuffed_zero_mask(x[i], prev);
            prev = x[i] >> 24;
        }
        if (markers) {
            const uint32_t behind = pieces == 4 ? (t < kThreads - 1 ? buf[(t + 1) * 17] & 0xFFu : behind_chunk) : 0x01u;
            prev = before_lane;
#pragma unroll
            for (uint32_t i = 0; i < 16; i++) {
                d[i] |= marker_mask(x[i], prev, i < 15 ? (x[i < 15 ? i + 1 : 15] & 0xFFu) : behind);
                prev = x[i] >> 24;
            }
        }
#pragma unroll
        for (uint32_t i = 0; i < 16; i++) {
            const uint32_t p = __popc(d[i]);
            n += p;
            gone[i / 5] |= p << (6 * (i % 5) + 3);
            const uint32_t m = __builtin_amdgcn_udot4(d[i], 0x08040201u, 0u, false) >> 7;
            x[i] = __builtin_amdgcn_perm(x[i], x[i], squeeze_sel[m]);
        }
    }
    uint32_t incl = n;
    for (int d = 1; d < 64; d <<= 1) {
        const uint32_t v = __shfl_up(incl, d);
        if ((t & 63) >= d) incl += v;
    }
    if ((t & 63) == 63) wave_base[t >> 6] = incl;
    __syncthreads();
    uint32_t excl = incl - n;
    for (int w = 0; w < (t >> 6); w++) excl += wave_base[w];
    const uint32_t chunk_drops = wave_base[0] + wave_base[1] + wave_base[2] + wave_base[3];
    auto padded = [](uint32_t k) { return k + ((k >> 6) << 2); };
    const uint32_t o0 = a + t * 64 - excl, cnt0 = o0 & 3;
    uint32_t slot = o0 >> 2, bits = 8 * cnt0, acc = 0;
    if (len) {
#pragma unroll
        for (uint32_t i = 0; i < 16; i++) {
            const unsigned long long w = (unsigned long long)x[i] << bits;
            const uint32_t p = (gone[i / 5] >> (6 * (i % 5))) & 63u;
            const bool full = bits >= p;
            acc |= (uint32_t)w;
            if (full) buf[slot + (slot >> 4)] = acc;
            acc = full ? (uint32_t)(w >> 32) : acc;
            slot += full ? 1u : 0u;
            bits = (bits - p) & 24u;
        }
    }
    const uint32_t o = slot * 4, cnt = bits / 8;
    __syncthreads();
    {
        const uint32_t from = slot == (o0 >> 2) ? cnt0 : 0u;
#pragma unroll
        for (uint32_t b = 0; b < 3; b++)
            if (b >= from && b < cnt) bytes[padded(o + b)] = (uint8_t)((uint32_t)acc >> (8 * b));
    }
    __syncthreads();
    const uint32_t n_out = chunk_len - chunk_drops;
    uint8_t* dst = const_cast<uint8_t*>(im.stream) + (gout - a);
    const uint32_t first_full = a ? 1 : 0, end_full = (a + n_out) / 4;
    for (uint32_t d = first_full + t; d < end_full; d += kThreads) reinterpret_cast<uint32_t*>(dst)[d] = buf[d + (d >> 4)];
    if (t < 4) {
        if (a && (uint32_t)t >= a && (uint32_t)t < a + n_out) dst[t] = bytes[padded((uint32_t)t)];
        const uint32_t tail = max(end_full, first_full) * 4 + t;
        if (tail >= a && tail < a + n_out && tail >= 4 * first_full) dst[tail] = bytes[padded(tail)];
    }
    if (chunk_begin + chunk_len == raw_bytes) {
        const uint32_t total = raw_bytes - before - chunk_drops;
        const uint32_t padded = ((total + 3) & ~3u) + kStreamSlackBytes;
        uint8_t* s = const_cast<uint8_t*>(im.stream);
        if (total + t < padded) s[total + t] = 0xFF;
        if (t == 0) {
            im.total_bits = total * 8;
            im.num_subseq = (total * 8 + kSubseqBits - 1) / kSubseqBits;
            im.stream_words = padded / 4;
        }
    }
}

__global__ __launch_bounds__(kSyncThreads) void huff_sync_kernel(const HuffImage* __restrict__ images, const HuffUnit* __restrict__ units,
                                                             unsigned long long* __restrict__ states, unsigned long long* __restrict__ incoming,
                                                             unsigned int* __restrict__ counters, int first_pass, int max_rounds,
                                                             uint16_t* __restrict__ tail_tasks, uint32_t* __restrict__ tail_count, uint16_t* records)
{
    __shared__ WgShared sh;
    extern __shared__ uint16_t dyn_pool[];
    HJ_LDS uint16_t* pool = (HJ_LDS uint16_t*)dyn_pool;
    const HuffUnit u = units[blockIdx.x];
    const HuffImage& im = images[u.image];
    const HuffGeom geom = make_geom(im);
    const uint32_t nsub = (geom.total_bits + kSubseqBits - 1) / kSubseqBits;
    if (u.first >= nsub) return;
    unsigned long long* gstate = states + im.first_subseq;
    const int t = threadIdx.x;
    const uint32_t j = u.first - 1 + t;
    const bool owner = t >= 1 && j < nsub;
    const int n_rows = (int)min((uint32_t)kSyncThreads, nsub - u.first + 1);
    unsigned long long in_state = 0;
    if (!first_pass) {
        in_state = u.first ? __hip_atomic_load(&gstate[u.first - 1], __ATOMIC_RELAXED, __HIP_MEMORY_SCOPE_AGENT) & kSyncMask : 0ull;
        if (in_state == incoming[blockIdx.x]) return;
    }
    stage_rows<kSyncThreads>(sh.stream, im, (int)u.first - 1);
    stage_pool<kSyncThreads>(pool, im);
    stage_constants(sh.tsel, nullptr, nullptr, im, false);
    __syncthreads();

    DevEnv env = make_env(sh, pool, u.first, geom, im);
    const bool rst = im.restart_interval != 0;
    unsigned long long old_global = ~0ull;
    int task = -1;
    const bool recording = !rst;
    if (first_pass) {
        const unsigned long long assumed = (unsigned long long)j * kSubseqBits;
        unsigned long long mine = 0;
        if (owner || (t == 0 && u.first > 0)) {
            const uint32_t bidx0 = boundary0_of(im, j);
            env.set_row(t);
            mine = pack_state(sync_walk(rst, false,geom, env, j * kSubseqBits, (j + 1) * kSubseqBits, 0, 0, bidx0, SlotRecorder()));
        }
        sh.end[t] = mine;
        __syncthreads();
        if (owner && ((sh.end[t - 1] & kSyncMask) != assumed || recording)) task = t;
    } else {
        if (owner) old_global = gstate[j];
        sh.end[t] = t == 0 ? in_state : old_global;
        if (t == 1) task = 1;
    }
    int rounds = 0;
    for (int round = 0; round < kSyncThreads + 2; round++) {
        __syncthreads();
        rounds++;
        unsigned long long now = 0;
        bool moved = false;
        if (task >= 0) {
            const SubseqState p = unpack_state(sh.end[task - 1]);
            env.set_row(task);
            const uint32_t jt = u.first - 1 + task;
            const SlotRecorder rec = slot_recorder(records, im, jt);
            const SubseqState st = sync_walk(rst, recording,geom, env, p.end_bit, (jt + 1) * kSubseqBits, p.zk & 255, p.zk >> 8, boundary0_of(im, jt), rec);
            if (recording) put_mark(rec, p.end_bit, (jt + 1) * kSubseqBits, geom.total_bits, p.zk & 255, st);
            now = pack_state(st);
            moved = ((now ^ sh.end[task]) & kSyncMask) != 0;
        }
        __syncthreads();
        if (task >= 0) sh.end[task] = now;
        const int pending = compact_tasks(sh, moved && task + 1 < n_rows, task + 1, &task);
        if (pending == 0 || rounds >= max_rounds) {
            if (tail_count) {
                if (t < pending) tail_tasks[(size_t)blockIdx.x * kSyncThreads + t] = (uint16_t)task;
                if (t == 0) tail_count[blockIdx.x] = (uint32_t)pending;
            }
            break;
        }
    }
    __syncthreads();
    if (owner) {
        const unsigned long long mine = sh.end[t];
        if (mine != old_global) {
            __hip_atomic_store(&gstate[j], mine, __ATOMIC_RELAXED, __HIP_MEMORY_SCOPE_AGENT);
            if (t == n_rows - 1 && ((mine ^ old_global) & kSyncMask) != 0) atomicAdd(counters + (first_pass ? 1 : 0), 1u);
        }
    }
    if (t == 0) {
        incoming[blockIdx.x] = first_pass ? (sh.end[0] & kSyncMask) : in_state;
        atomicAdd(counters + (first_pass ? 2 : 4), (unsigned)rounds);
        atomicMax(counters + (first_pass ? 3 : 5), (unsigned)rounds);
    }
}

constexpr int kTailWaves = 4;
constexpr int kTailThreads = 64 * kTailWaves;
#ifndef HJ_TAIL_SLOTS
#define HJ_TAIL_SLOTS 32
#endif
constexpr int kTailSlots = HJ_TAIL_SLOTS;
static_assert(kTailSlots == 32 || kTailSlots == 64, "a power of two, at most one row buffer per lane");
constexpr int kTailRowWords = kSubseqWords + 4;

struct TailWave {
    uint32_t rows[kTailSlots * kTailRowWords];
    uint16_t list[2][kSyncThreads];
    uint32_t count[2];
};
struct TailShared {
    TailWave wave[kTailWaves];
    uint32_t tsel[10];
};

struct TailEnv : LdsTables {
    uint32_t row_base;
    uint32_t word0;
    const uint32_t* boundaries;
    uint32_t num_boundaries;
    __device__ __forceinline__ uint32_t boundary(uint32_t i) const { return load_boundary(boundaries, num_boundaries, i); }
    static constexpr uint32_t kCursorStep = (uint32_t)kTailSlots * 4u;
    __device__ __forceinline__ uint32_t cursor(uint32_t i) const { return row_base + (i - word0) * kCursorStep; }
    __device__ __forceinline__ uint32_t fetch(uint32_t c) const { return *(const HJ_LDS uint32_t*)(uintptr_t)c; }
};
__device__ __forceinline__ SubseqState lane_walk(bool rst, bool record, const HuffGeom& geom, const TailEnv& env, uint32_t begin, uint32_t limit, int z, int k,
                                                 uint32_t boundary0, const SlotRecorder& rec)
{
    if (rst) return decode_subsequence<true>(geom, env, begin, limit, z, k, boundary0);
    return record ? decode_subsequence<false>(geom, env, begin, limit, z, k, 0, rec) : decode_subsequence<false>(geom, env, begin, limit, z, k);
}

__device__ __forceinline__ void wave_sync()
{
    __builtin_amdgcn_fence(__ATOMIC_ACQ_REL, "workgroup");
    __builtin_amdgcn_wave_barrier();
}


__device__ __forceinline__ unsigned long long state_in_front(const unsigned long long* states, const HuffImage& im, const HuffUnit u)
{
    return u.first ? __hip_atomic_load(&states[im.first_subseq + u.first - 1], __ATOMIC_RELAXED, __HIP_MEMORY_SCOPE_AGENT) & kSyncMask : 0ull;
}

__device__ __forceinline__ uint32_t uni(uint32_t v) { return (uint32_t)__builtin_amdgcn_readfirstlane((int)v); }
__device__ __forceinline__ uint32_t lane_read(uint32_t v, uint32_t lane) { return (uint32_t)__builtin_amdgcn_readlane((int)v, (int)lane); }

struct CoopWindow : LdsTables {
    const HJ_LDS uint32_t* row;
    uint32_t row_bit0, lane;
    uint32_t edc, eac;
    __device__ __forceinline__ uint32_t entry(uint32_t table, uint32_t w) const
    {
        uint32_t e = lookup1(table, w);
        if ((e >> 9) == kZadvLong) e = lookup2(e, w);
        return e;
    }
    __device__ __forceinline__ void open(uint32_t pos, uint32_t ts)
    {
        const uint32_t b = pos + lane - row_bit0, bit = b & 31u;
        const uint32_t w0 = row[(b >> 5) * kTailSlots], w1 = row[((b >> 5) + 1) * kTailSlots];
        const uint32_t w = bit ? __builtin_amdgcn_alignbit(w0, w1, 32u - bit) : w0;
        edc = entry(ts & 0xFFFFu, w);
        eac = entry(ts >> 16, w);
    }
    __device__ __forceinline__ uint32_t dc(uint32_t rel) const { return lane_read(edc, rel); }
    __device__ __forceinline__ uint32_t ac(uint32_t rel) const { return lane_read(eac, rel); }
};

constexpr int kTailRoundBudget = 192, kRippleRoundBudget = 192;
#ifndef HJ_COOP_CHAINS
#define HJ_COOP_CHAINS 2
#endif
constexpr int kCoopChains = HJ_COOP_CHAINS;
#ifndef HJ_TAIL_REENTRIES
#define HJ_TAIL_REENTRIES 4
// ... 720 lines not shown
    uint32_t until = lo < hi ? (seg == 0xFFFFFFFFu ? 0xFFFFFFFFu : (seg - lo % seg) % seg) : 0xFFFFFFFFu;
    for (uint32_t s = lo; s < hi; s += kBatch) {
        int d[kBatch];
#pragma unroll
        for (int i = 0; i < kBatch; i++) d[i] = s + i < hi ? (int)diff[index_of(s + i)] : 0;
#pragma unroll
        for (int i = 0; i < kBatch; i++) {
            if (s + i < hi) {
                if (until == 0) {
                    sum = 0;
                    flag = 1;
                    until = seg;
                }
                until--;
            }
            sum += d[i];
        }
    }
    s_sum[threadIdx.x] = sum;
    s_flag[threadIdx.x] = flag;
    __syncthreads();
    for (int off = 1; off < kThreads; off <<= 1) {
        int a = 0, fa = 0;
        if (threadIdx.x >= (unsigned)off) {
            a = s_sum[threadIdx.x - off];
            fa = s_flag[threadIdx.x - off];
        }
        __syncthreads();
        if (threadIdx.x >= (unsigned)off && !s_flag[threadIdx.x]) {
            s_sum[threadIdx.x] += a;
            s_flag[threadIdx.x] = fa;
        }
        __syncthreads();
    }
    int run = threadIdx.x ? s_sum[threadIdx.x - 1] : 0;
    until = lo < hi ? (seg == 0xFFFFFFFFu ? 0xFFFFFFFFu : (seg - lo % seg) % seg) : 0xFFFFFFFFu;
    for (uint32_t s = lo; s < hi; s += kBatch) {
        int d[kBatch];
#pragma unroll
        for (int i = 0; i < kBatch; i++) d[i] = s + i < hi ? (int)diff[index_of(s + i)] : 0;
#pragma unroll
        for (int i = 0; i < kBatch; i++) {
            if (s + i < hi) {
                if (until == 0) {
                    run = 0;
                    until = seg;
                }
                until--;
                run += d[i];
                const uint32_t mcu = (s + i) / bpc, jj = (s + i) - mcu * bpc;
                const uint32_t my = mcu / mcus_x, mx = mcu - my * mcus_x;
                const uint32_t dy = jj / h, dx = jj - dy * h;
                plane[(my * v + dy) * bw + (mx * h + dx)] = (int16_t)run;
            }
        }
    }
}

}

int launch_gather_raw(const HuffImage* images, const HuffUnit* chunk_units, int nchunks, void* stream)
{
    if (nchunks <= 0) return 0;
    hipLaunchKernelGGL(gather_raw_kernel, dim3(min(nchunks, kGatherGroups)), dim3(kThreads), 0, (hipStream_t)stream, images, chunk_units, nchunks);
    return (int)hipGetLastError();
}

int launch_destuff(HuffImage* images, const HuffUnit* chunk_units, int nchunks, uint32_t* drops, bool count_on_device, unsigned int* counters,
                   void* stream)
{
    if (nchunks <= 0) return 0;
    if (count_on_device)
        hipLaunchKernelGGL(destuff_count_kernel, dim3(nchunks), dim3(kThreads), 0, (hipStream_t)stream, images, chunk_units, drops);
    hipLaunchKernelGGL(destuff_compact_kernel, dim3(nchunks), dim3(kThreads), 0, (hipStream_t)stream, images, chunk_units, drops, counters);
    return (int)hipGetLastError();
}

static bool ripple_in_tail_kernel()
{
    static const bool v = getenv("HIPJPEG_RIPPLE_IN_SYNC") == nullptr;
    return v;
}

int launch_huff_sync(HuffImage* images, const HuffUnit* units, int nunits, unsigned long long* states, unsigned long long* incoming,
                     unsigned int* changed, int first_pass, int max_rounds, uint16_t* tail_tasks, uint32_t* tail_count, uint16_t* records,
                     unsigned pool_bytes, void* stream, unsigned pass_id)
{
    if (nunits <= 0) return 0;
    const dim3 tail_grid((nunits + kTailWaves - 1) / kTailWaves);
    if (!first_pass && ripple_in_tail_kernel()) {
        hipLaunchKernelGGL(huff_tail_kernel<true>, tail_grid, dim3(kTailThreads), pool_bytes, (hipStream_t)stream, images, units, nunits, states, incoming,
                           changed, nullptr, nullptr, pass_id, records);
        return (int)hipGetLastError();
    }
    hipLaunchKernelGGL(huff_sync_kernel, dim3(nunits), dim3(kSyncThreads), pool_bytes, (hipStream_t)stream, images, units, states, incoming, changed,
                       first_pass, max_rounds, tail_tasks, tail_count, records);
    if (tail_count)
        hipLaunchKernelGGL(huff_tail_kernel<false>, tail_grid, dim3(kTailThreads), pool_bytes, (hipStream_t)stream, images, units, nunits, states, incoming,
                           changed, tail_tasks, tail_count, 0u, records);
    return (int)hipGetLastError();
}

int launch_huff_write(HuffImage* images, const HuffUnit* sync_units, int nsync_units, const HuffUnit* block_units, int nblock_units,
                      const unsigned long long* states, uint32_t* first_block, const uint16_t* records, uint32_t* walkers, int32_t* group_sums,
                      unsigned pool_bytes, void* stream, bool dc_only)
{
    if (nsync_units <= 0) return 0;
    hipLaunchKernelGGL(huff_copy_records_kernel, dim3(nsync_units), dim3(kSyncThreads), 0, (hipStream_t)stream, images, sync_units, states, first_block,
                       records, walkers);
    hipLaunchKernelGGL(huff_pos_kernel, dim3(nsync_units), dim3(kSyncThreads), pool_bytes, (hipStream_t)stream, images, sync_units, states, first_block,
                       records, walkers);
    if (nblock_units > 0) {
        if (dc_only)
            hipLaunchKernelGGL(huff_dcdiff_kernel, dim3(nblock_units), dim3(kThreads), 0, (hipStream_t)stream, images, block_units, group_sums);
        else
            hipLaunchKernelGGL(huff_blocks_kernel, dim3((nblock_units + kBTeams - 1) / kBTeams * kBTeams), dim3(kBThreads), pool_bytes, (hipStream_t)stream,
                               images, block_units, (uint32_t)nblock_units, group_sums);
    }
    return (int)hipGetLastError();
}

int launch_huff_dc(const HuffImage* images, const HuffUnit* rst_units, int nrst_units, const HuffUnit* block_units, int nblock_units,
                   const int32_t* group_sums, const unsigned int* counters, unsigned int* verdicts, void* stream)
{
    if (nblock_units > 0)
        hipLaunchKernelGGL(huff_dc_group_kernel, dim3(nblock_units), dim3(kThreads), 0, (hipStream_t)stream, images, block_units, group_sums, counters,
                           verdicts);
    if (nrst_units > 0) hipLaunchKernelGGL(huff_dc_kernel, dim3(nrst_units), dim3(kThreads), 0, (hipStream_t)stream, images, rst_units);
    return (int)hipGetLastError();
}

}
```

### nvimagecodec_amd/csrc/gpu_huffman_host.cpp

```cpp
#include "gpu_huffman_host.h"
#include "scratch_fill.h"

#include <algorithm>
#include <cstring>

namespace hipjpeg {

uint32_t scan_mcus_x(const FrameInfo& f, const ScanHeader& sc)
{
    return (uint32_t)(sc.ncomp == 1 ? (f.comp[sc.comp_index[0]].samp_w + 7) / 8 : f.mcus_x);
}

uint32_t scan_mcus_y(const FrameInfo& f, const ScanHeader& sc)
{
    return (uint32_t)(sc.ncomp == 1 ? (f.comp[sc.comp_index[0]].samp_h + 7) / 8 : f.mcus_y);
}

uint32_t scan_blocks_per_mcu(const FrameInfo& f, const ScanHeader& sc)
{
    if (sc.ncomp == 1) return 1;
    uint32_t n = 0;
    for (int i = 0; i < sc.ncomp; i++) n += (uint32_t)(f.comp[sc.comp_index[i]].h * f.comp[sc.comp_index[i]].v);
    return n;
}
// ... 222 lines not shown
        for (int dy = 0; dy < v; dy++)
            for (int dx = 0; dx < h; dx++, k++) {
                HuffK& hk = im->k[k];
                hk.comp = (uint8_t)i;
                hk.blk0 = (uint32_t)(dy * fc.blocks_w + dx);
                hk.stride_y = (uint32_t)(v * fc.blocks_w);
                hk.stride_x = (uint8_t)h;
            }
    }
    im->blocks_per_mcu = (uint32_t)k;
    im->total_blocks = im->mcus_x * im->mcus_y * (uint32_t)k;
}

namespace {
struct HostEnv {
    const HuffImage* im;
    static constexpr uint32_t kCursorStep = 1;
    uint32_t cursor(uint32_t i) const { return i; }
    uint32_t fetch(uint32_t i) const { return word(i); }
    uint32_t word(uint32_t i) const
    {
        const uint8_t* p = im->stream + (size_t)i * 4;
        return i < im->stream_words ? ((uint32_t)p[0] << 24) | ((uint32_t)p[1] << 16) | ((uint32_t)p[2] << 8) | (uint32_t)p[3] : ~0u;
    }
    uint32_t boundary(uint32_t i) const { return i < im->num_boundaries ? im->boundaries[i] : 0xFFFFFFFFu; }
    uint32_t lookup1(uint32_t t, uint32_t w) const { return im->pool[t + (w >> (32 - kHuffFastBits))]; }
    uint32_t lookup2(uint32_t e, uint32_t w) const { return im->pool[(e & 0x1FFu) * 64u + ((w >> 16) & ((1u << kHuffSubBits) - 1))]; }
    uint32_t lookup_pair(uint32_t t, uint32_t w) const
    {
        const size_t i = (size_t)t + kPairOffset + (w >> (32 - kHuffFastBits));
        return i < im->pool_words ? im->pool[i] : 0u;
    }
    uint32_t tables(int k) const { return (uint32_t)im->k[k].tdc | ((uint32_t)im->k[k].tac << 16); }
    int16_t* block_ptr(int k, uint32_t mx, uint32_t my) const
    {
        const HuffK& hk = im->k[k];
        return im->coef[hk.comp] + ((size_t)hk.blk0 + (size_t)my * hk.stride_y + (size_t)mx * hk.stride_x) * 64;
    }
    int zigzag(int z) const { return kZigzagDeviceGpuHost[z]; }
    int16_t* buf;
    void put(int index, int value) const { buf[index] = (int16_t)value; }
    StepTables step;
    void step_tables(uint32_t d, uint32_t* tdc, uint32_t* tac) const { select_halves<true>(step, d, tdc, tac); }
    uint32_t step_entry(uint32_t t, uint32_t w) const { return lookup1(t, w); }
    uint32_t step_pair(uint32_t t, uint32_t w) const { return lookup_pair(t, w); }
    uint32_t step_second(uint32_t e) const { return second_table_of(e, 6u, 0u); }
};

struct HostWindow {
    const HostEnv* env;
    uint32_t edc[64], eac[64];
    uint32_t tables(uint32_t k) const { return env->tables((int)k); }
    uint32_t entry(uint32_t table, uint32_t w) const
    {
        uint32_t e = env->lookup1(table, w);
        if ((e >> 9) == kZadvLong) e = env->lookup2(e, w);
        return e;
    }
    void open(uint32_t pos, uint32_t ts)
    {
        for (uint32_t l = 0; l < 64; l++) {
            const uint32_t b = pos + l, bit = b & 31u;
            const uint32_t w0 = env->word(b >> 5), w1 = env->word((b >> 5) + 1);
            const uint32_t w = bit ? (w0 << bit) | (w1 >> (32u - bit)) : w0;
            edc[l] = entry(ts & 0xFFFFu, w);
            eac[l] = entry(ts >> 16, w);
        }
    }
    uint32_t dc(uint32_t rel) const { return edc[rel]; }
    uint32_t ac(uint32_t rel) const { return eac[rel]; }
};

struct HostRecorder {
    uint16_t* rec;
    uint32_t bit0;
    void operator()(uint32_t i, uint32_t pos) const
    {
        rec[i < (uint32_t)kRecSlots ? i : (uint32_t)kRecSlots] = (uint16_t)(pos - bit0);
    }
};
}

namespace {
int emulate_scan(const uint8_t* data, const FrameInfo& f, const ScanHeader& sc, int16_t* const frame_coef[4], int* sync_passes)
{
    std::vector<uint8_t> stream = device_scratch<uint8_t>(destuffed_capacity(sc));
    const size_t n = destuff_scan(data, sc, stream.data());
    std::vector<uint16_t> pool(gpu_pool_words(sc));
    HuffImage im;
    fill_huff_image(f, sc, (uint32_t)n, &im);
    build_gpu_pool(sc, &im, pool.data());
    std::vector<int16_t> dc_diff = device_scratch<int16_t>(im.total_blocks);
    std::vector<uint32_t> boundaries;
    for (uint32_t b : sc.rst_after) boundaries.push_back(b * 8u);
    im.stream = stream.data();
    im.pool = pool.data();
    im.dc_diff = dc_diff.data();
    im.boundaries = boundaries.data();
    im.num_boundaries = (uint32_t)boundaries.size();
    im.restart_interval = (uint32_t)sc.restart_interval;
    const bool rst = sc.restart_interval != 0;
    for (int i = 0; i < sc.ncomp; i++) {
        const int c = sc.comp_index[i];
        int16_t* const coef = frame_coef[c];
        im.coef[i] = coef;
        const size_t bw = (size_t)f.comp[c].blocks_w, bh = (size_t)f.comp[c].blocks_h, rows = sc.ncomp == 1 ? im.mcus_y : bh;
        const size_t cols = sc.ncomp == 1 ? im.mcus_x : bw;
        if (sc.ncomp == 1 && (im.mcus_x < bw || im.mcus_y < bh)) {
            const size_t first = im.mcus_x < bw ? 0 : (size_t)im.mcus_y * bw;
            memset(coef + first * 64, 0, (bw * bh - first) * 128);
        }
        for (size_t y = 0; y < rows; y++) memset(coef + y * bw * 64, 0x5A, cols * 128);
    }
    int16_t block_buffer[64] = {0};
    HostEnv env{&im, block_buffer, StepTables()};
    {
        const TableClasses classes = make_countdown_classes(im.blocks_per_mcu, [&](uint32_t q) { return env.tables((int)q); });
        if (!classes.complete) return 5;
        env.step = split_classes(classes, 1u, 0u);
        for (uint32_t q = 0; q < im.blocks_per_mcu; q++) {
            uint32_t tdc, tac;
            env.step_tables(im.blocks_per_mcu - 1u - q, &tdc, &tac);
            if ((tdc | (tac << 16)) != env.tables((int)q)) return 5;
        }
    }
    const HuffGeom geom = make_geom(im);
    const uint32_t ns = im.num_subseq;
    std::vector<SubseqState> cur = device_scratch<SubseqState>(ns), nxt = device_scratch<SubseqState>(ns);
    uint32_t err = 0;
    std::vector<uint16_t> records = device_scratch<uint16_t>((size_t)ns * kRecShorts);
    bool forms_differ = false;
    uint16_t other[kRecShorts];
    auto walk = [&](uint32_t i, uint32_t begin, int z, int k, bool record) {
        const uint32_t limit = (i + 1) * kSubseqBits;
        uint16_t* rec = &records[(size_t)i * kRecShorts];
        SubseqState st, sb;
        uint32_t mark = kRecInvalid;
        size_t named = 0;
        if (rst) {
            st = select_walk<true>(geom, env, begin, limit, z, k, 0);
            sb = decode_subsequence<true>(geom, env, begin, limit, z, k, 0);
        } else if (!record) {
            st = select_walk<false>(geom, env, begin, limit, z, k);
            sb = decode_subsequence<false>(geom, env, begin, limit, z, k);
        } else {
            st = select_walk<false>(geom, env, begin, limit, z, k, 0, HostRecorder{rec, i * kSubseqBits});
            sb = decode_subsequence<false>(geom, env, begin, limit, z, k, 0, HostRecorder{other, i * kSubseqBits});
            mark = record_mark(begin, limit < geom.total_bits ? limit : geom.total_bits, (uint32_t)z, st);
            named = mark_valid(mark) ? 2 * (mark & (kRecFresh - 1)) : 0;
        }
        if (pack_state(st) != pack_state(sb) || memcmp(other, rec, named) != 0) forms_differ = true;
        rec[kRecMark] = (uint16_t)mark;
        return st;
    };
    for (uint32_t i = 0; i < ns; i++) cur[i] = walk(i, i * kSubseqBits, 0, 0, i == 0);
    int passes = 0;
    for (;;) {
        bool changed = false;
        if (ns) nxt[0] = cur[0];
        for (uint32_t i = 1; i < ns; i++) {
            const SubseqState& prev = cur[i - 1];
            nxt[i] = walk(i, prev.end_bit, prev.zk & 255, prev.zk >> 8, true);
            if (pack_state(nxt[i]) != pack_state(cur[i])) changed = true;
        }
        cur.swap(nxt);
        passes++;
        if (!changed) break;
        if (passes > (int)ns + 2) return 3;
    }
    if (sync_passes) *sync_passes = passes;
    if (forms_differ) return 5;
    if (!rst) {
        HostWindow win;
        win.env = &env;
        const uint32_t changes = cooperative_table_changes(win, geom.blocks_per_mcu);
        std::vector<uint16_t> coop(kRecShorts), lane(kRecShorts);
        for (uint32_t i = 0; i < ns; i++) {
            const uint32_t begin = i ? cur[i - 1].end_bit : 0u, z = i ? (cur[i - 1].zk & 255u) : 0u, k = i ? (uint32_t)(cur[i - 1].zk >> 8) : 0u;
            const uint32_t limit = (i + 1) * kSubseqBits, end = limit < geom.total_bits ? limit : geom.total_bits;
            const uint16_t* final_rec = &records[(size_t)i * kRecShorts];
            const SubseqState cs = cooperative_subsequence(geom, win, changes, begin, limit, z, k, HostRecorder{coop.data(), i * kSubseqBits});
            if (pack_state(cs) != pack_state(cur[i])) return 4;
            const uint32_t final_mark = final_rec[kRecMark];
            if (record_mark(begin, end, z, cs) != final_mark) return 5;
            if (mark_valid(final_mark) && memcmp(coop.data(), final_rec, 2 * (final_mark & (kRecFresh - 1))) != 0) return 5;
            const SubseqState cg = cooperative_subsequence(geom, win, changes, i * kSubseqBits, limit, 0, 0, HostRecorder{coop.data(), i * kSubseqBits});
            const SubseqState lg = decode_subsequence<false>(geom, env, i * kSubseqBits, limit, 0, 0, 0, HostRecorder{lane.data(), i * kSubseqBits});
            if (pack_state(cg) != pack_state(lg)) return 4;
            const uint32_t mark = record_mark(i * kSubseqBits, end, 0, lg);
            if (mark_valid(mark) && memcmp(coop.data(), lane.data(), 2 * (mark & (kRecFresh - 1))) != 0) return 5;
        }
    }
    std::vector<uint32_t> first_block = device_scratch<uint32_t>(ns);
    uint32_t acc = 0;
    for (uint32_t i = 0; i < ns; i++) {
        first_block[i] = acc;
        acc += cur[i].nblocks;
    }
    if (acc < im.total_blocks) return 2;
    std::vector<uint32_t> block_pos(im.total_blocks, 0xFFFFFFFFu);
    std::vector<uint32_t> found_block, found_pos;
    for (uint32_t i = 0; i < ns; i++) {
        const uint32_t begin = i == 0 ? 0 : cur[i - 1].end_bit;
        const int z = i == 0 ? 0 : (cur[i - 1].zk & 255), k = i == 0 ? 0 : (cur[i - 1].zk >> 8);
        found_block.clear();
        found_pos.clear();
        auto rec = [&](uint32_t block, uint32_t pos) {
            found_block.push_back(block);
            found_pos.push_back(pos);
            if (block < im.total_blocks) block_pos[block] = pos;
        };
        if (rst) {
            uint32_t fault = 0;
            position_subsequence<true>(geom, env, begin, (i + 1) * kSubseqBits, z, k, first_block[i], rec, 0, &fault);
            if (fault) return 1;
        } else
            position_subsequence<false>(geom, env, begin, (i + 1) * kSubseqBits, z, k, first_block[i], rec);
        const uint16_t* r = &records[(size_t)i * kRecShorts];
        const uint32_t mark = r[kRecMark];
        if (rst || !mark_valid(mark)) {
            if (!rst && mark != kRecOverflow) return 5;
            if (mark == kRecOverflow && found_block.size() <= (size_t)kRecSlots) return 5;
            continue;
        }
        const uint32_t n = mark & (kRecFresh - 1), b0 = first_block[i] + ((mark & kRecFresh) ? 0u : 1u);
        if (n != found_block.size()) return 5;
        for (uint32_t s = 0; s < n; s++)
            if (found_block[s] != b0 + s || found_pos[s] != i * kSubseqBits + r[s]) return 5;
    }
    if (geom.interval_blocks)
        for (uint32_t j = 0; j < im.num_boundaries && (uint64_t)(j + 1) * geom.interval_blocks < im.total_blocks; j++)
            if (block_pos[(j + 1) * geom.interval_blocks] != im.boundaries[j]) return 1;
    for (uint32_t b = 0; b < im.total_blocks; b++) {
        if (block_pos[b] == 0xFFFFFFFFu) return 2;
        int k;
        int16_t* dst = block_address(geom, env, b, &k);
        memset(block_buffer, 0, sizeof block_buffer);
        dc_diff[b] = (int16_t)decode_block(geom, env, block_pos[b], k, &err);
        memcpy(dst, block_buffer, 128);
    }
    if (err) return 1;
    int pred[4] = {0, 0, 0, 0};
    uint32_t block = 0, mcu = 0;
    for (uint32_t my = 0; my < im.mcus_y; my++)
        for (uint32_t mx = 0; mx < im.mcus_x; mx++, mcu++) {
            if (rst && mcu % im.restart_interval == 0) pred[0] = pred[1] = pred[2] = pred[3] = 0;
            for (uint32_t k = 0; k < im.blocks_per_mcu; k++, block++) {
                const int c = im.k[k].comp;
                pred[c] += dc_diff[block];
                env.block_ptr((int)k, mx, my)[0] = (int16_t)pred[c];
            }
        }
    return 0;
}
}

int emulate_gpu_entropy(const uint8_t* data, size_t size, const FrameInfo& f, int16_t* const coef[4], int* sync_passes)
{
    (void)size;
    for (int c = 0; c < f.ncomp; c++) fill_device_scratch(coef[c], (size_t)f.comp[c].blocks_w * f.comp[c].blocks_h * 128);
    int passes = 0;
    for (const ScanHeader& sc : f.scans) {
        int p = 0;
        const int rc = emulate_scan(data, f, sc, coef, &p);
        passes = std::max(passes, p);
        if (rc != 0) return rc;
    }
    if (sync_passes) *sync_passes = passes;
    return 0;
}

}
```

### nvimagecodec_amd/csrc/gpu_huffman_host.h

```cpp
#pragma once
#include <cstddef>
#include <cstdint>
#include <vector>

#include "huffman_gpu_core.h"
#include "jpeg_syntax.h"

namespace hipjpeg {

constexpr int kMaxSeqScans = 4;
bool gpu_entropy_eligible(const FrameInfo& f);

uint32_t scan_mcus_x(const FrameInfo& f, const ScanHeader& sc);
uint32_t scan_mcus_y(const FrameInfo& f, const ScanHeader& sc);
uint32_t scan_blocks_per_mcu(const FrameInfo& f, const ScanHeader& sc);

inline size_t destuffed_capacity(const ScanHeader& sc) { return (((sc.data_end - sc.data_begin) + 3) & ~(size_t)3) + kStreamSlackBytes; }

size_t destuff_scan(const uint8_t* data, const ScanHeader& sc, uint8_t* out);

size_t gpu_pool_words(const ScanHeader& sc);

void build_gpu_pool(const ScanHeader& sc, HuffImage* im, uint16_t* pool);

bool pair_table_steps(const HuffSpec& ac, uint32_t* out);

void fill_huff_image(const FrameInfo& f, const ScanHeader& sc, uint32_t stream_bytes, HuffImage* im);

int emulate_gpu_entropy(const uint8_t* data, size_t size, const FrameInfo& f, int16_t* const coef[4], int* sync_passes);

}
```

### nvimagecodec_amd/csrc/hipjpeg_api.cpp

```cpp
#include <hip/hip_runtime_api.h>

#include <cstring>
#include <memory>
#include <new>
#include <vector>

#include "../../include/hipjpeg.h"
#include "coefficients_core.h"
#include "decoder_core.h"
#include "diagnostics.h"
#include "encoder_core.h"
#include "entropy_decode.h"
#include "gpu_huffman_encode.h"
#include "gpu_huffman_host.h"
#include "lossless_batch.h"
#include "progressive_encode.h"
#include "progressive_gpu_host.h"
#include "scratch_fill.h"
#include "thread_pool.h"
#include "transcode_core.h"

#include <chrono>
#include <future>
#include <cstdio>
// ... 135 lines not shown
    }
    info->coef_bytes = f.total_blocks() * 128;
    return HIPJPEG_STATUS_SUCCESS;
    });
}

hipjpegStatus_t hipjpegEntropyDecodeHost(const uint8_t* data, size_t length, int16_t* coef, size_t coef_capacity_bytes,
                                         uint64_t comp_offsets[4], uint16_t qtables[256])
{
    return guarded([&]() -> hipjpegStatus_t {
    if (!data || !coef) return HIPJPEG_STATUS_INVALID_ARGUMENT;
    FrameInfo f;
    ParseStatus ps = parse_jpeg(data, length, &f);
    if (ps != kParseOk) return status_from_parse(ps);
    if (f.total_blocks() * 128 > coef_capacity_bytes) return HIPJPEG_STATUS_BUFFER_TOO_SMALL;
    int16_t* ptr[4] = {nullptr, nullptr, nullptr, nullptr};
    size_t off = 0;
    for (int c = 0; c < f.ncomp; c++) {
        ptr[c] = coef + off;
        if (comp_offsets) comp_offsets[c] = off;
        off += (size_t)f.comp[c].blocks_w * f.comp[c].blocks_h * 64;
        if (qtables)
            for (int j = 0; j < 64; j++) qtables[c * 64 + (j & 7) * 8 + (j >> 3)] = f.qtab[c][j];
    }
    switch (decode_coefficients(data, length, f, ptr)) {
    case kEntropyOk: return HIPJPEG_STATUS_SUCCESS;
    case kEntropyTruncated: return HIPJPEG_STATUS_TRUNCATED;
    case kEntropyMissingTable: return HIPJPEG_STATUS_BAD_JPEG;
    default: return HIPJPEG_STATUS_CORRUPT;
    }
    });
}

hipjpegStatus_t hipjpegEntropyDecodeHostSparse(const uint8_t* data, size_t length, uint8_t* stream, size_t capacity_bytes, size_t* stream_bytes,
                                               uint64_t table_offsets[4])
{
    return guarded([&]() -> hipjpegStatus_t {
    if (!data || !stream || !stream_bytes) return HIPJPEG_STATUS_INVALID_ARGUMENT;
    FrameInfo f;
    ParseStatus ps = parse_jpeg(data, length, &f);
    if (ps != kParseOk) return status_from_parse(ps);
    if (!sparse_staging_applies(f)) return HIPJPEG_STATUS_UNSUPPORTED;
    if (sparse_stream_capacity(f) > capacity_bytes) return HIPJPEG_STATUS_BUFFER_TOO_SMALL;
    size_t blocks = 0;
    for (int c = 0; c < f.ncomp; c++) {
        if (table_offsets) table_offsets[c] = blocks;
        blocks += (size_t)f.comp[c].blocks_w * f.comp[c].blocks_h;
    }
    switch (decode_coefficients_sparse(data, length, f, stream, stream_bytes)) {
    case kEntropyOk: return HIPJPEG_STATUS_SUCCESS;
    case kEntropyTruncated: return HIPJPEG_STATUS_TRUNCATED;
    case kEntropyMissingTable: return HIPJPEG_STATUS_BAD_JPEG;
    default: return HIPJPEG_STATUS_CORRUPT;
    }
    });
}

hipjpegStatus_t hipjpegEntropyDecodeGpuAlgorithmHost(const uint8_t* data, size_t length, int16_t* coef, size_t coef_capacity_bytes,
                                                     uint64_t comp_offsets[4], int32_t* sync_passes)
{
    return guarded([&]() -> hipjpegStatus_t {
    if (!data || !coef) return HIPJPEG_STATUS_INVALID_ARGUMENT;
    FrameInfo f;
    ParseStatus ps = parse_jpeg(data, length, &f);
    if (ps != kParseOk) return status_from_parse(ps);
    const bool progressive = gpu_progressive_eligible(f);
    if (!progressive && !gpu_entropy_eligible(f)) return HIPJPEG_STATUS_UNSUPPORTED;
    if (f.total_blocks() * 128 > coef_capacity_bytes) return HIPJPEG_STATUS_BUFFER_TOO_SMALL;
    int16_t* ptr[4] = {nullptr, nullptr, nullptr, nullptr};
    size_t off = 0;
    for (int c = 0; c < f.ncomp; c++) {
        ptr[c] = coef + off;
        if (comp_offsets) comp_offsets[c] = off;
        off += (size_t)f.comp[c].blocks_w * f.comp[c].blocks_h * 64;
    }
    int passes = 0;
    int rc = progressive ? emulate_gpu_progressive(data, length, f, ptr) : emulate_gpu_entropy(data, length, f, ptr, &passes);
    if (sync_passes) *sync_passes = passes;
    if (rc == 5) return HIPJPEG_STATUS_INTERNAL_ERROR;
    return rc == 0 ? HIPJPEG_STATUS_SUCCESS : (rc == 2 ? HIPJPEG_STATUS_TRUNCATED : HIPJPEG_STATUS_CORRUPT);
    });
}

hipjpegStatus_t hipjpegEntropyDecodeGpuIntervalAlgorithmHost(const uint8_t* data, size_t length, int16_t* coef, size_t coef_capacity_bytes,
                                                             uint64_t comp_offsets[4])
{
    return guarded([&]() -> hipjpegStatus_t {
    if (!data || !coef) return HIPJPEG_STATUS_INVALID_ARGUMENT;
    FrameInfo f;
    ParseStatus ps = parse_jpeg(data, length, &f);
    if (ps != kParseOk) return status_from_parse(ps);
    if (!gpu_progressive_interval_eligible(f)) return HIPJPEG_STATUS_UNSUPPORTED;
    if (f.total_blocks() * 128 > coef_capacity_bytes) return HIPJPEG_STATUS_BUFFER_TOO_SMALL;
    int16_t* ptr[4] = {nullptr, nullptr, nullptr, nullptr};
    size_t off = 0;
    for (int c = 0; c < f.ncomp; c++) {
        ptr[c] = coef + off;
        if (comp_offsets) comp_offsets[c] = off;
        off += (size_t)f.comp[c].blocks_w * f.comp[c].blocks_h * 64;
    }
    return emulate_gpu_progressive_intervals(data, length, f, ptr) == 0 ? HIPJPEG_STATUS_SUCCESS : HIPJPEG_STATUS_CORRUPT;
    });
}

hipjpegStatus_t hipjpegCreate(hipjpegHandle_t* handle, int device_id, int num_host_threads)
{
    return guarded([&]() -> hipjpegStatus_t {
    if (!handle) return HIPJPEG_STATUS_INVALID_ARGUMENT;
    *handle = nullptr;
    int count = 0;
    if (hipGetDeviceCount(&count) != hipSuccess || count <= 0) return HIPJPEG_STATUS_NO_DEVICE;
    if (device_id < 0 || device_id >= count) return HIPJPEG_STATUS_INVALID_ARGUMENT;
    hipjpegHandle* h = new (std::nothrow) hipjpegHandle();
    if (!h) return HIPJPEG_STATUS_ALLOC_FAILED;
    h->device_id = device_id;
    h->pool.reset(new ForkJoinPool(num_host_threads));
    for (auto& b : h->batches) b.reset(new DecodeBatch(device_id, &h->hooks));
    h->encode.reset(new EncodeBatch(device_id, &h->hooks));
    h->encode_view = h->encode.get();
    *handle = h;
    return HIPJPEG_STATUS_SUCCESS;
    });
}

hipjpegStatus_t hipjpegDestroy(hipjpegHandle_t handle)
{
    return guarded([&]() -> hipjpegStatus_t {
    if (!handle) return HIPJPEG_STATUS_INVALID_ARGUMENT;
    (void)hipSetDevice(handle->device_id);
    if (handle->copy_stream) (void)hipStreamDestroy(handle->copy_stream);
    if (handle->entropy_stream) (void)hipStreamDestroy(handle->entropy_stream);
    for (hipStream_t ps : handle->page_entropy_stream)
        if (ps) (void)hipStreamDestroy(ps);
    for (auto& pg : handle->encode_pages) {
        if (pg.result.valid()) {
            try {
                (void)pg.result.get();
            } catch (...) {
            }
        }
        pg.batch.reset();
        if (pg.ready) (void)hipEventDestroy(pg.ready);
        if (pg.stream) (void)hipStreamDestroy(pg.stream);
    }
    delete handle;
    return HIPJPEG_STATUS_SUCCESS;
    });
}

hipjpegStatus_t hipjpegDecodeBatchHost(hipjpegHandle_t handle, const uint8_t* const* data, const size_t* lengths, int batch_size,
                                       const hipjpegOutput_t* outputs, hipjpegOutputFormat_t format, unsigned flags,
                                       hipjpegStatus_t* statuses)
{
    return guarded([&]() -> hipjpegStatus_t {
    if (!handle) return HIPJPEG_STATUS_INVALID_ARGUMENT;
    handle->current = (handle->current + 1) % handle->pages;
    handle->settled = -1;
    DecodeBatch& b = handle->cur();
    static const bool timing = getenv("HIPJPEG_DEBUG_TIMING") != nullptr;
    const auto t0 = std::chrono::steady_clock::now();
    const bool geometry = !handle->transforms.empty(), scaled = !handle->scales.empty();
    if ((geometry && (int)handle->transforms.size() != batch_size) || (scaled && (int)handle->scales.size() != batch_size)) {
        handle->transforms.clear();
        handle->scales.clear();
        return HIPJPEG_STATUS_INVALID_ARGUMENT;
    }
// ... 799 lines not shown
```

### nvimagecodec_amd/lowlevel.py

```python
import ctypes

import numpy as np

from . import _native as N

_FORMATS = {"rgb": N.OUTPUT_RGBI, "bgr": N.OUTPUT_BGRI, "rgb_planar": N.OUTPUT_RGB_PLANAR, "bgr_planar": N.OUTPUT_BGR_PLANAR,
            "y": N.OUTPUT_Y, "yuv_planar": N.OUTPUT_YUV_PLANAR}


def _as_u8(data):
    if isinstance(data, np.ndarray):
        return np.ascontiguousarray(data, dtype=np.uint8)
    if hasattr(data, "data_ptr") and hasattr(data, "numpy"):
        return data.numpy()
    return np.frombuffer(bytes(data), dtype=np.uint8)


def entropy_decode_host_sparse(data):
    a = _as_u8(data)
    info = get_image_info(data)
    nblocks = [bh * bw for bh, bw in zip(info["blocks_h"], info["blocks_w"])]
    cap = sum(nblocks) * 200 + 64
    buf = np.zeros(cap, dtype=np.uint8)
    n = ctypes.c_size_t()
    toff = (ctypes.c_uint64 * 4)()
    st = N.load().hipjpegEntropyDecodeHostSparse(a.ctypes.data, a.size, buf.ctypes.data, cap, ctypes.byref(n), toff)
    if st:
        raise N.HipJpegError(st, "hipjpegEntropyDecodeHostSparse")
    tables = buf[: sum(nblocks) * 4].view(np.uint32)
    out = []
    for c, nb in enumerate(nblocks):
        blocks = np.zeros((nb, 64), dtype=np.int16)
        for b in range(nb):
            off = int(tables[int(toff[c]) + b])
            if off == 0:
                continue
            k = int(buf[off])
            blocks[b, 0] = np.frombuffer(buf[off + 1:off + 3].tobytes(), dtype="<i2")[0]
            for e in range(k):
                r = off + 3 + 3 * e
                blocks[b, int(buf[r])] = np.frombuffer(buf[r + 1:r + 3].tobytes(), dtype="<i2")[0]
        blk = blocks.reshape(info["blocks_h"][c], info["blocks_w"][c], 8, 8)
        out.append(np.ascontiguousarray(blk.transpose(0, 1, 3, 2)).reshape(info["blocks_h"][c], info["blocks_w"][c], 64))
    return out, int(n.value)


def set_twin_scratch_fill(byte):
    st = N.load().hipjpegTestSetScratchFill(int(byte))
    if st:
        raise N.HipJpegError(st, "hipjpegTestSetScratchFill")


def get_image_info(data):
    a = _as_u8(data)
    info = N.ImageInfo()
    st = N.load().hipjpegGetImageInfo(a.ctypes.data, a.size, ctypes.byref(info))
    if st:
        raise N.HipJpegError(st, "hipjpegGetImageInfo")
    nc = info.num_components
    d = {k: getattr(info, k) for k in ("width", "height", "num_components", "sof_marker", "color_model", "subsampling",
                                        "restart_interval", "num_scans", "coef_bytes")}
    for k in ("h", "v", "blocks_w", "blocks_h", "samp_w", "samp_h"):
        d[k] = list(getattr(info, k))[:nc]
    return d


def entropy_decode_host(data):
    a = _as_u8(data)
    info = get_image_info(a)
    buf = np.zeros(info["coef_bytes"] // 2, dtype=np.int16)
    offs = (ctypes.c_uint64 * 4)()
    qt = np.zeros(256, dtype=np.uint16)
    st = N.load().hipjpegEntropyDecodeHost(a.ctypes.data, a.size, buf.ctypes.data, buf.nbytes, ctypes.addressof(offs), qt.ctypes.data)
    if st:
        raise N.HipJpegError(st, "hipjpegEntropyDecodeHost")
    coefs, qts = [], []
    for c in range(info["num_components"]):
        n = info["blocks_w"][c] * info["blocks_h"][c]
        blk = buf[offs[c]: offs[c] + n * 64].reshape(info["blocks_h"][c], info["blocks_w"][c], 8, 8)
        coefs.append(np.ascontiguousarray(blk.transpose(0, 1, 3, 2)).reshape(info["blocks_h"][c], info["blocks_w"][c], 64))
        qts.append(np.ascontiguousarray(qt[c * 64:(c + 1) * 64].reshape(8, 8).T).reshape(64))
    return coefs, qts


def entropy_decode_gpu_algorithm_host(data):
    a = _as_u8(data)
    info = get_image_info(a)
    buf = np.zeros(info["coef_bytes"] // 2, dtype=np.int16)
    offs = (ctypes.c_uint64 * 4)()
    passes = ctypes.c_int32()
    st = N.load().hipjpegEntropyDecodeGpuAlgorithmHost(a.ctypes.data, a.size, buf.ctypes.data, buf.nbytes, ctypes.addressof(offs), ctypes.byref(passes))
    if st:
        raise N.HipJpegError(st, "hipjpegEntropyDecodeGpuAlgorithmHost")
    coefs = []
    for c in range(info["num_components"]):
        n = info["blocks_w"][c] * info["blocks_h"][c]
        blk = buf[offs[c]: offs[c] + n * 64].reshape(info["blocks_h"][c], info["blocks_w"][c], 8, 8)
        coefs.append(np.ascontiguousarray(blk.transpose(0, 1, 3, 2)).reshape(info["blocks_h"][c], info["blocks_w"][c], 64))
    return coefs, passes.value


def entropy_decode_gpu_interval_algorithm_host(data):
    a = _as_u8(data)
    info = get_image_info(a)
    buf = np.zeros(info["coef_bytes"] // 2, dtype=np.int16)
    offs = (ctypes.c_uint64 * 4)()
    st = N.load().hipjpegEntropyDecodeGpuIntervalAlgorithmHost(a.ctypes.data, a.size, buf.ctypes.data, buf.nbytes, ctypes.addressof(offs))
    if st:
        raise N.HipJpegError(st, "hipjpegEntropyDecodeGpuIntervalAlgorithmHost")
    coefs = []
    for c in range(info["num_components"]):
        n = info["blocks_w"][c] * info["blocks_h"][c]
        blk = buf[offs[c]: offs[c] + n * 64].reshape(info["blocks_h"][c], info["blocks_w"][c], 8, 8)
        coefs.append(np.ascontiguousarray(blk.transpose(0, 1, 3, 2)).reshape(info["blocks_h"][c], info["blocks_w"][c], 64))
    return coefs


def _decode_flags(fancy, gpu_huffman, fast_idct, gpu_progressive_intervals=False):
    return ((N.FLAG_FANCY_UPSAMPLING if fancy else 0) | (N.FLAG_GPU_HUFFMAN if gpu_huffman else 0) | (N.FLAG_FAST_IDCT if fast_idct else 0) |
            (N.FLAG_GPU_PROGRESSIVE_INTERVALS if gpu_progressive_intervals else 0))


def scaled_image_size(width, height, scale_denom):
    w, h = ctypes.c_int32(), ctypes.c_int32()
    st = N.load().hipjpegGetScaledImageSize(int(width), int(height), int(scale_denom), ctypes.byref(w), ctypes.byref(h))
    if st:
        raise N.HipJpegError(st, "hipjpegGetScaledImageSize")
    return w.value, h.value


def output_shapes(jpegs, fmt="rgb", transforms=None, scales=None):
    shapes = []
    for i, j in enumerate(jpegs):
        try:
            info = get_image_info(j)
            h, w = info["height"], info["width"]
            if scales is not None and scales[i] != 1:
                w, h = scaled_image_size(w, h, scales[i])
        except N.HipJpegError:
            shapes.append(None)
            continue
        if transforms is not None and transforms[i] is not None:
            roi, orientation = transforms[i]
            if roi is not None:
                w, h = roi[2] - roi[0], roi[3] - roi[1]
            if orientation >= 5:
                w, h = h, w
        if fmt in ("rgb", "bgr"):
            shapes.append((h, w, 3))
        elif fmt in ("rgb_planar", "bgr_planar"):
            shapes.append((3, h, w))
        elif fmt == "y":
            shapes.append((h, w))
        else:
            shapes.append([(info["samp_h"][c], info["samp_w"][c]) for c in range(min(info["num_components"], 3))])
    return shapes


def _set_allocators(handle, allocators):
    if allocators is None:
        return None
    table = allocators.hipjpeg_allocators() if hasattr(allocators, "hipjpeg_allocators") else allocators
    st = N.load().hipjpegSetAllocators(handle, ctypes.byref(table))
    if st:
        raise N.HipJpegError(st, "hipjpegSetAllocators")
    return (allocators, table)


class BatchDecoder:

    def __init__(self, device=0, num_threads=0, allocators=None):
        import torch
        self._torch = torch
        self.device = int(device)
        self._h = ctypes.c_void_p()
        st = N.load().hipjpegCreate(ctypes.byref(self._h), self.device, int(num_threads))
        if st:
            raise N.HipJpegError(st, "hipjpegCreate")
        self._allocators = _set_allocators(self._h, allocators)
        self._keep = None
        self._inflight = []

# ... 1040 lines not shown
```

Baseline: 117,300.

## Pair adjacent Huffman sync units in one first-pass workgroup kernel

Adds a paired first-pass sync kernel in which each workgroup stages two adjacent sync units (2*kHuffOwn+1 rows). The second unit's first subsequence can then start from the first unit's real end state instead of a guessed bit offset. The aim is fewer resynchronisation rounds and fewer later ripple passes for sequential-scan Huffman decode. It costs larger LDS use per workgroup, a pair table uploaded to the device, a split of the old sync kernel into first-pass and later-pass variants, and a host emulator plus test hook that count schedule phases.

Measured after the change: 125,300 (median of 6 runs). 6.9% higher.

```diff
diff --git a/include/hipjpeg.h b/include/hipjpeg.h
--- a/include/hipjpeg.h
+++ b/include/hipjpeg.h
@@ -84,6 +84,8 @@
 
 HIPJPEG_API int32_t hipjpegTestScanChunkDrops(const uint8_t* data, size_t length, int scan_index, uint32_t* drops, int32_t capacity);
 HIPJPEG_API int32_t hipjpegTestPairSteps(const uint8_t bits[16], const uint8_t* vals, int32_t nvals, uint32_t* steps);
+
+HIPJPEG_API hipjpegStatus_t hipjpegTestSyncScheduleCounts(const uint8_t* data, size_t length, uint64_t counts[10]);
 
 HIPJPEG_API hipjpegStatus_t hipjpegTestSetScratchFill(int byte);
 
diff --git a/nvimagecodec_amd/csrc/decoder_core.cpp b/nvimagecodec_amd/csrc/decoder_core.cpp
--- a/nvimagecodec_amd/csrc/decoder_core.cpp
+++ b/nvimagecodec_amd/csrc/decoder_core.cpp
@@ -303,7 +303,7 @@
     host_fallback_images_ = 0;
     xform_desc_.clear();
     prog_slot_words_ = 0;
-    max_huff_units_ = max_pool_words_ = 0;
+    max_huff_units_ = max_huff_pairs_ = max_pool_words_ = 0;
     coef_bytes_ = output_bytes_ = 0;
     if (pool_ && n > 1)
         pool_->parallel_for(n, [&](int i, int) { prepare(i, a); });
@@ -596,7 +596,9 @@
         const size_t nsub = (s.scan(sc, &q.raw_offset, &q.stream_offset, &q.first_chunk) * 8 + kSubseqBits - 1) / kSubseqBits;
         const size_t mcus = (size_t)scan_mcus_x(f, sc) * scan_mcus_y(f, sc);
         s.subseq += nsub;
-        max_huff_units_ += std::max<size_t>((nsub + kHuffOwn - 1) / kHuffOwn, 1);
+        const size_t sync_units = std::max<size_t>((nsub + kHuffOwn - 1) / kHuffOwn, 1);
+        max_huff_units_ += sync_units;
+        max_huff_pairs_ += (sync_units + 1) / 2;
         q.pool_words = gpu_pool_words(sc);
         q.tables_offset = s.pools.take(align_up(q.pool_words * 2, 64), 1);
         max_pool_words_ = std::max(max_pool_words_, q.pool_words);
@@ -616,6 +618,7 @@
     L.units = c.take(sizeof(WorkUnit) * s.units);
     L.huff_desc = c.take(sizeof(HuffImage) * (ng + s.prog_scans));
     L.huff_units = c.take(sizeof(HuffUnit) * max_huff_units_);
+    L.huff_pairs = c.take(sizeof(uint32_t) * max_huff_pairs_);
     L.huff_wunits = c.take(sizeof(HuffUnit) * s.huff_wunits);
     L.huff_dc_units = c.take(sizeof(HuffUnit) * ng * 4);
     L.huff_chunk_units = c.take(sizeof(HuffUnit) * chunks);
@@ -939,6 +942,7 @@
 void DecodeBatch::build_entropy_units()
 {
     for (std::vector<HuffUnit>* v : {&huff_units_, &huff_wunits_, &huff_chunk_units_, &huff_dc_units_, &prog_units_}) v->clear();
+    huff_pairs_.clear();
     uint32_t first_subseq = 0;
     stream_bytes_total_ = 0;
     huff_zero_.clear();
@@ -980,7 +984,9 @@
         }
         h.first_subseq = first_subseq;
         first_subseq += h.num_subseq;
+        const size_t first_unit = huff_units_.size();
         for (uint32_t j = 0; j == 0 || j < h.num_subseq; j += kHuffOwn) huff_units_.push_back(HuffUnit{(uint32_t)g, j});
+        for (size_t i = first_unit; i < huff_units_.size(); i += 2) huff_pairs_.push_back(huff_pair_entry((uint32_t)i, i + 1 < huff_units_.size()));
         if (h.restart_interval)
             for (uint32_t i = 0; i < h.ncomp; i++) huff_dc_units_.push_back(HuffUnit{(uint32_t)g, i});
         stream_bytes_total_ += q.stream_bytes;
@@ -1140,6 +1146,7 @@
     copy_table(pinned_, staging_.prog_iv_units, prog_iv_units_);
     copy_table(pinned_, staging_.huff_desc, huff_images_);
     copy_table(pinned_, staging_.huff_units, huff_units_);
+    copy_table(pinned_, staging_.huff_pairs, huff_pairs_);
     copy_table(pinned_, staging_.huff_wunits, huff_wunits_);
     copy_table(pinned_, staging_.huff_dc_units, huff_dc_units_);
     copy_table(pinned_, staging_.huff_chunk_units, huff_chunk_units_);
@@ -1218,10 +1225,11 @@
     static const int tail_after = getenv("HIPJPEG_TAIL_AFTER") ? atoi(getenv("HIPJPEG_TAIL_AFTER")) : 2;
     uint16_t* tail_tasks = at<uint16_t>(work_, scratch_.tail);
     uint32_t* tail_count = at<uint32_t>(work_, scratch_.tail + (size_t)max_huff_units_ * kTailTaskBytes);
-    if (launch_huff_sync(L.dimg, L.dunits, L.nunits, L.states, L.incoming, L.changed, 1, tail_after > 0 ? tail_after : 1 << 20,
+    if (launch_huff_sync(L.dimg, L.dunits, L.nunits, at<const uint32_t>(device_, staging_.huff_pairs), (int)huff_pairs_.size(), L.states, L.incoming,
+                         L.changed, 1, tail_after > 0 ? tail_after : 1 << 20,
                          tail_after > 0 ? tail_tasks : nullptr, tail_after > 0 ? tail_count : nullptr, L.records, L.pool_bytes, stream) != 0)
         return HIPJPEG_STATUS_HIP_ERROR;
-    if (launch_huff_sync(L.dimg, L.dunits, L.nunits, L.states, L.incoming, L.changed, 0, 1 << 20, nullptr, nullptr, L.records, L.pool_bytes, stream, 1) != 0)
+    if (launch_huff_sync(L.dimg, L.dunits, L.nunits, nullptr, 0, L.states, L.incoming, L.changed, 0, 1 << 20, nullptr, nullptr, L.records, L.pool_bytes, stream, 1) != 0)
         return HIPJPEG_STATUS_HIP_ERROR;
     if (!entropy_write_passes(L, stream)) return HIPJPEG_STATUS_HIP_ERROR;
     if (L.verdicts_out != L.host_changed && hipMemcpyAsync(L.host_changed, L.verdicts_out, verdict_bytes(), hipMemcpyDeviceToHost, s) != hipSuccess)
@@ -1337,7 +1345,7 @@
         from_desc = true;
         for (int pass = 0; pass < kExtraRippleLaunches && !converged; pass++) {
             if (hipMemsetAsync(L.changed, 0, sizeof(unsigned int), s) != hipSuccess) return HIPJPEG_STATUS_HIP_ERROR;
-            if (launch_huff_sync(L.dimg, L.dunits, L.nunits, L.states, L.incoming, L.changed, 0, 1 << 20, nullptr, nullptr, L.records, L.pool_bytes, stream, ++last_pass) != 0)
+            if (launch_huff_sync(L.dimg, L.dunits, L.nunits, nullptr, 0, L.states, L.incoming, L.changed, 0, 1 << 20, nullptr, nullptr, L.records, L.pool_bytes, stream, ++last_pass) != 0)
                 return HIPJPEG_STATUS_HIP_ERROR;
             if (hipMemcpyAsync(L.host_changed, L.changed, sizeof(unsigned int), hipMemcpyDeviceToHost, s) != hipSuccess) return HIPJPEG_STATUS_HIP_ERROR;
             if (hipStreamSynchronize(s) != hipSuccess) return HIPJPEG_STATUS_HIP_ERROR;
diff --git a/nvimagecodec_amd/csrc/decoder_core.h b/nvimagecodec_amd/csrc/decoder_core.h
--- a/nvimagecodec_amd/csrc/decoder_core.h
+++ b/nvimagecodec_amd/csrc/decoder_core.h
@@ -149,7 +149,7 @@
     Buffer export_pinned_, export_device_;
     uint64_t exported_blocks_ = 0;
     struct StagingLayout {
-        size_t desc, units, huff_desc, huff_units, huff_wunits, huff_dc_units, huff_chunk_units, huff_drops, xform_desc, xform_units,
+        size_t desc, units, huff_desc, huff_units, huff_pairs, huff_wunits, huff_dc_units, huff_chunk_units, huff_drops, xform_desc, xform_units,
             prog_desc, prog_units, prog_iv_desc, prog_iv_units, tensor_planes, tensor_units, tables, boundaries, streams, coef, h2d_bytes, gpu_coef_begin, total;
     } staging_{};
     struct WorkLayout {
@@ -178,6 +178,7 @@
     std::vector<TransformImage> xform_desc_;
     std::vector<HuffImage> huff_images_;
     std::vector<HuffUnit> huff_units_, huff_dc_units_;
+    std::vector<uint32_t> huff_pairs_;
     std::vector<int> huff_to_image_;
     int seq_gpu_images_ = 0;
     struct ZeroFill {
@@ -187,7 +188,7 @@
     std::vector<ZeroFill> huff_zero_;
     std::vector<HuffUnit> huff_wunits_;
     std::vector<HuffUnit> huff_chunk_units_;
-    size_t total_subseq_ = 0, max_huff_units_ = 0, max_pool_words_ = 0;
+    size_t total_subseq_ = 0, max_huff_units_ = 0, max_huff_pairs_ = 0, max_pool_words_ = 0;
     std::atomic<bool> host_drops_missing_{false};
     std::vector<ProgImage> prog_images_;
     std::vector<int> prog_to_image_;
diff --git a/nvimagecodec_amd/csrc/gpu_huffman.h b/nvimagecodec_amd/csrc/gpu_huffman.h
--- a/nvimagecodec_amd/csrc/gpu_huffman.h
+++ b/nvimagecodec_amd/csrc/gpu_huffman.h
@@ -14,9 +14,10 @@
 int launch_destuff(HuffImage* images, const HuffUnit* chunk_units, int nchunks, uint32_t* drops, bool count_on_device, unsigned int* counters,
                    void* stream);
 
-int launch_huff_sync(HuffImage* images, const HuffUnit* units, int nunits, unsigned long long* states, unsigned long long* incoming,
-                     unsigned int* changed, int first_pass, int max_rounds, uint16_t* tail_tasks, uint32_t* tail_count, uint16_t* records,
-                     unsigned pool_bytes, void* stream, unsigned pass_id = 0);
+constexpr uint32_t huff_pair_entry(uint32_t first_unit, bool with_next) { return first_unit | (with_next ? 0x80000000u : 0u); }
+int launch_huff_sync(HuffImage* images, const HuffUnit* units, int nunits, const uint32_t* pairs, int npairs, unsigned long long* states,
+                     unsigned long long* incoming, unsigned int* changed, int first_pass, int max_rounds, uint16_t* tail_tasks, uint32_t* tail_count,
+                     uint16_t* records, unsigned pool_bytes, void* stream, unsigned pass_id = 0);
 int launch_huff_write(HuffImage* images, const HuffUnit* sync_units, int nsync_units, const HuffUnit* block_units, int nblock_units,
                       const unsigned long long* states, uint32_t* first_block, const uint16_t* records, uint32_t* walkers,
                       int32_t* group_sums, unsigned pool_bytes, void* stream, bool dc_only = false);
diff --git a/nvimagecodec_amd/csrc/gpu_huffman.hip b/nvimagecodec_amd/csrc/gpu_huffman.hip
--- a/nvimagecodec_amd/csrc/gpu_huffman.hip
+++ b/nvimagecodec_amd/csrc/gpu_huffman.hip
@@ -1,4 +1,6 @@
 #include <hip/hip_runtime.h>
+
+#include <type_traits>
 
 #include "gpu_huffman.h"
 #include "huffman_gpu_core.h"
@@ -30,6 +32,17 @@
     uint32_t queue[kSyncThreads];
     uint32_t wave_count[kSyncThreads / 64];
 };
+
+constexpr int kPairRows = 2 * kHuffOwn + 1;
+struct PairShared {
+    uint32_t stream[staged_lds_words(kSyncThreads)];
+    unsigned long long end[2 * kSyncThreads];
+    unsigned long long second_from;
+    uint32_t tsel[10];
+    uint32_t wave_count[kSyncThreads / 64];
+    uint16_t queue[kSyncThreads];
+};
+static_assert(kSyncThreads != 256 || sizeof(PairShared) + 13824 <= 53760, "huff_sync_pair_kernel: three workgroups per CU");
 
 __device__ __forceinline__ uint32_t load_boundary(const uint32_t* boundaries, uint32_t n, uint32_t i)
 {
@@ -88,6 +101,11 @@
         row_addr = stream_base + ((uint32_t)row << 2);
         row_word0 = word0 + ((uint32_t)row << kRowShift);
     }
+    __device__ __forceinline__ void set_column_row(int column, int row)
+    {
+        row_addr = stream_base + ((uint32_t)column << 2);
+        row_word0 = word0 + ((uint32_t)row << kRowShift);
+    }
     __device__ __forceinline__ uint32_t cursor(uint32_t i) const { return row_addr + (i - row_word0) * kCursorStep; }
     __device__ __forceinline__ uint32_t fetch(uint32_t c) const { return *(const HJ_LDS uint32_t*)(uintptr_t)c; }
 };
@@ -141,12 +159,12 @@
 }
 
 template <int ROWS>
-__device__ __forceinline__ void stage_rows(uint32_t* lds_stream, const HuffImage& im, int first_row)
+__device__ __forceinline__ void stage_row(uint32_t* lds_stream, const HuffImage& im, int row)
 {
     const int t = threadIdx.x;
     const HJ_GLOBAL uint32_t* g = (const HJ_GLOBAL uint32_t*)im.stream;
     const int nwords = (int)im.stream_words;
-    const int w0 = (first_row + t) * kSubseqWords;
+    const int w0 = row * kSubseqWords;
     constexpr int kGroups = kSubseqWords / 4;
     u32x4 v[kGroups];
     typedef unsigned int u32x2 __attribute__((ext_vector_type(2)));
@@ -174,6 +192,11 @@
     }
     dst[(kSubseqWords + 0) * ROWS] = __builtin_bswap32(tail.x);
     dst[(kSubseqWords + 1) * ROWS] = __builtin_bswap32(tail.y);
+}
+template <int ROWS>
+__device__ __forceinline__ void stage_rows(uint32_t* lds_stream, const HuffImage& im, int first_row)
+{
+    stage_row<ROWS>(lds_stream, im, first_row + (int)threadIdx.x);
 }
 
 template <int THREADS>
@@ -212,7 +235,8 @@
     }
 }
 
-__device__ __forceinline__ DevEnv make_env(WgShared& sh, HJ_LDS uint16_t* pool, uint32_t first, const HuffGeom& geom, const HuffImage& im)
+template <class Shared>
+__device__ __forceinline__ DevEnv make_env(Shared& sh, HJ_LDS uint16_t* pool, uint32_t first, const HuffGeom& geom, const HuffImage& im)
 {
     DevEnv env;
     env.stream_base = (uint32_t)(uintptr_t)(HJ_LDS uint32_t*)sh.stream;
@@ -227,7 +251,8 @@
     return env;
 }
 
-__device__ __forceinline__ int compact_tasks(WgShared& sh, bool has, int value, int* task)
+template <class Shared>
+__device__ __forceinline__ int compact_tasks(Shared& sh, bool has, int value, int* task)
 {
     const int t = threadIdx.x;
     const unsigned long long mask = __ballot(has);
@@ -241,7 +266,7 @@
         if (w < (t >> 6)) base += c;
         n += c;
     }
-    if (has) sh.queue[base + below] = (uint32_t)value;
+    if (has) sh.queue[base + below] = (std::remove_reference_t<decltype(sh.queue[0])>)value;
     __syncthreads();
     *task = t < n ? (int)sh.queue[t] : -1;
     return n;
@@ -495,8 +520,7 @@
 
 __global__ __launch_bounds__(kSyncThreads) void huff_sync_kernel(const HuffImage* __restrict__ images, const HuffUnit* __restrict__ units,
                                                              unsigned long long* __restrict__ states, unsigned long long* __restrict__ incoming,
-                                                             unsigned int* __restrict__ counters, int first_pass, int max_rounds,
-                                                             uint16_t* __restrict__ tail_tasks, uint32_t* __restrict__ tail_count, uint16_t* records)
+                                                             unsigned int* __restrict__ counters, uint16_t* records)
 {
     __shared__ WgShared sh;
     extern __shared__ uint16_t dyn_pool[];
@@ -511,11 +535,8 @@
     const uint32_t j = u.first - 1 + t;
     const bool owner = t >= 1 && j < nsub;
     const int n_rows = (int)min((uint32_t)kSyncThreads, nsub - u.first + 1);
-    unsigned long long in_state = 0;
-    if (!first_pass) {
-        in_state = u.first ? __hip_atomic_load(&gstate[u.first - 1], __ATOMIC_RELAXED, __HIP_MEMORY_SCOPE_AGENT) & kSyncMask : 0ull;
-        if (in_state == incoming[blockIdx.x]) return;
-    }
+    const unsigned long long in_state = u.first ? __hip_atomic_load(&gstate[u.first - 1], __ATOMIC_RELAXED, __HIP_MEMORY_SCOPE_AGENT) & kSyncMask : 0ull;
+    if (in_state == incoming[blockIdx.x]) return;
     stage_rows<kSyncThreads>(sh.stream, im, (int)u.first - 1);
     stage_pool<kSyncThreads>(pool, im);
     stage_constants(sh.tsel, nullptr, nullptr, im, false);
@@ -523,25 +544,10 @@
 
     DevEnv env = make_env(sh, pool, u.first, geom, im);
     const bool rst = im.restart_interval != 0;
-    unsigned long long old_global = ~0ull;
-    int task = -1;
     const bool recording = !rst;
-    if (first_pass) {
-        const unsigned long long assumed = (unsigned long long)j * kSubseqBits;
-        unsigned long long mine = 0;
-        if (owner || (t == 0 && u.first > 0)) {
-            const uint32_t bidx0 = boundary0_of(im, j);
-            env.set_row(t);
-            mine = pack_state(sync_walk(rst, false,geom, env, j * kSubseqBits, (j + 1) * kSubseqBits, 0, 0, bidx0, SlotRecorder()));
-        }
-        sh.end[t] = mine;
-        __syncthreads();
-        if (owner && ((sh.end[t - 1] & kSyncMask) != assumed || recording)) task = t;
-    } else {
-        if (owner) old_global = gstate[j];
-        sh.end[t] = t == 0 ? in_state : old_global;
-        if (t == 1) task = 1;
-    }
+    const unsigned long long old_global = owner ? gstate[j] : ~0ull;
+    sh.end[t] = t == 0 ? in_state : old_global;
+    int task = t == 1 ? 1 : -1;
     int rounds = 0;
     for (int round = 0; round < kSyncThreads + 2; round++) {
         __syncthreads();
@@ -553,34 +559,120 @@
             env.set_row(task);
             const uint32_t jt = u.first - 1 + task;
             const SlotRecorder rec = slot_recorder(records, im, jt);
-            const SubseqState st = sync_walk(rst, recording,geom, env, p.end_bit, (jt + 1) * kSubseqBits, p.zk & 255, p.zk >> 8, boundary0_of(im, jt), rec);
+            const SubseqState st = sync_walk(rst, recording, geom, env, p.end_bit, (jt + 1) * kSubseqBits, p.zk & 255, p.zk >> 8, boundary0_of(im, jt), rec);
             if (recording) put_mark(rec, p.end_bit, (jt + 1) * kSubseqBits, geom.total_bits, p.zk & 255, st);
             now = pack_state(st);
             moved = ((now ^ sh.end[task]) & kSyncMask) != 0;
         }
         __syncthreads();
         if (task >= 0) sh.end[task] = now;
-        const int pending = compact_tasks(sh, moved && task + 1 < n_rows, task + 1, &task);
-        if (pending == 0 || rounds >= max_rounds) {
-            if (tail_count) {
-                if (t < pending) tail_tasks[(size_t)blockIdx.x * kSyncThreads + t] = (uint16_t)task;
-                if (t == 0) tail_count[blockIdx.x] = (uint32_t)pending;
-            }
-            break;
-        }
+        if (compact_tasks(sh, moved && task + 1 < n_rows, task + 1, &task) == 0) break;
     }
     __syncthreads();
     if (owner) {
         const unsigned long long mine = sh.end[t];
         if (mine != old_global) {
             __hip_atomic_store(&gstate[j], mine, __ATOMIC_RELAXED, __HIP_MEMORY_SCOPE_AGENT);
-            if (t == n_rows - 1 && ((mine ^ old_global) & kSyncMask) != 0) atomicAdd(counters + (first_pass ? 1 : 0), 1u);
+            if (t == n_rows - 1 && ((mine ^ old_global) & kSyncMask) != 0) atomicAdd(counters + 0, 1u);
         }
     }
     if (t == 0) {
-        incoming[blockIdx.x] = first_pass ? (sh.end[0] & kSyncMask) : in_state;
-        atomicAdd(counters + (first_pass ? 2 : 4), (unsigned)rounds);
-        atomicMax(counters + (first_pass ? 3 : 5), (unsigned)rounds);
+        incoming[blockIdx.x] = in_state;
+        atomicAdd(counters + 4, (unsigned)rounds);
+        atomicMax(counters + 5, (unsigned)rounds);
+    }
+}
+
+__global__ __launch_bounds__(kSyncThreads) void huff_sync_pair_kernel(const HuffImage* __restrict__ images, const HuffUnit* __restrict__ units,
+                                                                  const uint32_t* __restrict__ pairs, unsigned long long* __restrict__ states,
+                                                                  unsigned long long* __restrict__ incoming, unsigned int* __restrict__ counters,
+                                                                  int max_rounds, uint16_t* __restrict__ tail_tasks, uint32_t* __restrict__ tail_count,
+                                                                  uint16_t* records)
+{
+    __shared__ PairShared sh;
+    extern __shared__ uint16_t dyn_pool[];
+    HJ_LDS uint16_t* pool = (HJ_LDS uint16_t*)dyn_pool;
+    const uint32_t pair = pairs[blockIdx.x];
+    const uint32_t ui = pair & 0x7FFFFFFFu;
+    const HuffUnit u = units[ui];
+    const HuffImage& im = images[u.image];
+    const HuffGeom geom = make_geom(im);
+    const uint32_t nsub = (geom.total_bits + kSubseqBits - 1) / kSubseqBits;
+    if (u.first >= nsub) return;
+    unsigned long long* gstate = states + im.first_subseq;
+    const int t = threadIdx.x;
+    const int n_rows = (int)min((uint32_t)((pair >> 31) ? kPairRows : kSyncThreads), nsub - u.first + 1);
+    const bool second = n_rows > kSyncThreads;
+    const auto subseq_of = [&](int row) { return u.first - 1 + (uint32_t)row; };
+    const bool in_a = 2 * t < n_rows && (t > 0 || u.first > 0);
+    if (in_a) stage_row<kSyncThreads>(sh.stream, im, (int)subseq_of(2 * t));
+    stage_pool<kSyncThreads>(pool, im);
+    stage_constants(sh.tsel, nullptr, nullptr, im, false);
+    __syncthreads();
+
+    DevEnv env = make_env(sh, pool, u.first, geom, im);
+    const bool rst = im.restart_interval != 0;
+    const bool recording = !rst;
+    const auto decode = [&](int row, unsigned long long from, bool record) {
+        const SubseqState p = unpack_state(from);
+        const uint32_t jt = subseq_of(row);
+        env.set_column_row(t, row);
+        const SlotRecorder rec = slot_recorder(records, im, jt);
+        const SubseqState st = sync_walk(rst, record, geom, env, p.end_bit, (jt + 1) * kSubseqBits, p.zk & 255, p.zk >> 8, boundary0_of(im, jt), rec);
+        if (record) put_mark(rec, p.end_bit, (jt + 1) * kSubseqBits, geom.total_bits, p.zk & 255, st);
+        return pack_state(st);
+    };
+    unsigned long long mine = 0;
+#pragma unroll 1
+    for (int ph = 0; ph < 2; ph++) {
+        const int row = 2 * t + ph;
+        const bool active = ph ? row < n_rows : in_a;
+        if (active) {
+            if (ph) stage_row<kSyncThreads>(sh.stream, im, (int)subseq_of(row));
+            const unsigned long long from = ph ? mine : (unsigned long long)subseq_of(row) * kSubseqBits;
+            if (row == kSyncThreads) sh.second_from = from & kSyncMask;
+            mine = decode(row, from, ph && recording);
+        }
+        if (active || row == 0) sh.end[row] = mine;
+    }
+    __syncthreads();
+    int task = -1;
+    if (t >= 1 && 2 * t < n_rows && (recording || (sh.end[2 * t - 1] & kSyncMask) != (unsigned long long)subseq_of(2 * t) * kSubseqBits)) task = 2 * t;
+    int rounds = 0, pending = 0;
+    for (int round = 0; round < kPairRows + 2; round++) {
+        rounds++;
+        bool moved = false;
+        if (task >= 0) {
+            stage_row<kSyncThreads>(sh.stream, im, (int)subseq_of(task));
+            const unsigned long long from = sh.end[task - 1];
+            if (task == kSyncThreads) sh.second_from = from & kSyncMask;
+            const unsigned long long now = decode(task, from, recording);
+            moved = ((now ^ sh.end[task]) & kSyncMask) != 0;
+            sh.end[task] = now;
+        }
+        pending = compact_tasks(sh, moved && task + 1 < n_rows, task + 1, &task);
+        if (pending == 0 || rounds >= max_rounds) break;
+    }
+    if (tail_count) {
+        const int n_first = __syncthreads_count(task >= 0 && task < kSyncThreads);
+        const int skip = n_first < pending && sh.queue[n_first] == kSyncThreads ? 1 : 0;
+        if (task >= 0 && task < kSyncThreads) tail_tasks[(size_t)ui * kSyncThreads + t] = (uint16_t)task;
+        if (task > kSyncThreads) tail_tasks[(size_t)(ui + 1) * kSyncThreads + (t - n_first - skip)] = (uint16_t)(task - kHuffOwn);
+        if (t == 0) {
+            tail_count[ui] = (uint32_t)n_first;
+            if (second) tail_count[ui + 1] = (uint32_t)(pending - n_first - skip);
+        }
+    }
+#pragma unroll
+    for (int row = t; row < 2 * kSyncThreads; row += kSyncThreads)
+        if (row >= 1 && row < n_rows) __hip_atomic_store(&gstate[subseq_of(row)], sh.end[row], __ATOMIC_RELAXED, __HIP_MEMORY_SCOPE_AGENT);
+    if (t == 0) {
+        const unsigned n_units = second ? 2u : 1u;
+        incoming[ui] = sh.end[0] & kSyncMask;
+        if (second) incoming[ui + 1] = sh.second_from;
+        atomicAdd(counters + 1, n_units);
+        atomicAdd(counters + 2, (unsigned)rounds * n_units);
+        atomicMax(counters + 3, (unsigned)rounds);
     }
 }
 
@@ -1467,19 +1559,23 @@
     return v;
 }
 
-int launch_huff_sync(HuffImage* images, const HuffUnit* units, int nunits, unsigned long long* states, unsigned long long* incoming,
-                     unsigned int* changed, int first_pass, int max_rounds, uint16_t* tail_tasks, uint32_t* tail_count, uint16_t* records,
-                     unsigned pool_bytes, void* stream, unsigned pass_id)
-{
-    if (nunits <= 0) return 0;
+int launch_huff_sync(HuffImage* images, const HuffUnit* units, int nunits, const uint32_t* pairs, int npairs, unsigned long long* states,
+                     unsigned long long* incoming, unsigned int* changed, int first_pass, int max_rounds, uint16_t* tail_tasks, uint32_t* tail_count,
+                     uint16_t* records, unsigned pool_bytes, void* stream, unsigned pass_id)
+{
+    if (nunits <= 0 || (first_pass && npairs <= 0)) return 0;
     const dim3 tail_grid((nunits + kTailWaves - 1) / kTailWaves);
     if (!first_pass && ripple_in_tail_kernel()) {
         hipLaunchKernelGGL(huff_tail_kernel<true>, tail_grid, dim3(kTailThreads), pool_bytes, (hipStream_t)stream, images, units, nunits, states, incoming,
                            changed, nullptr, nullptr, pass_id, records);
         return (int)hipGetLastError();
     }
-    hipLaunchKernelGGL(huff_sync_kernel, dim3(nunits), dim3(kSyncThreads), pool_bytes, (hipStream_t)stream, images, units, states, incoming, changed,
-                       first_pass, max_rounds, tail_tasks, tail_count, records);
+    if (first_pass)
+        hipLaunchKernelGGL(huff_sync_pair_kernel, dim3(npairs), dim3(kSyncThreads), pool_bytes, (hipStream_t)stream, images, units, pairs, states, incoming,
+                           changed, max_rounds, tail_tasks, tail_count, records);
+    else
+        hipLaunchKernelGGL(huff_sync_kernel, dim3(nunits), dim3(kSyncThreads), pool_bytes, (hipStream_t)stream, images, units, states, incoming, changed,
+                           records);
     if (tail_count)
         hipLaunchKernelGGL(huff_tail_kernel<false>, tail_grid, dim3(kTailThreads), pool_bytes, (hipStream_t)stream, images, units, nunits, states, incoming,
                            changed, tail_tasks, tail_count, 0u, records);
diff --git a/nvimagecodec_amd/csrc/gpu_huffman_host.cpp b/nvimagecodec_amd/csrc/gpu_huffman_host.cpp
--- a/nvimagecodec_amd/csrc/gpu_huffman_host.cpp
+++ b/nvimagecodec_amd/csrc/gpu_huffman_host.cpp
@@ -328,7 +328,59 @@
 }
 
 namespace {
-int emulate_scan(const uint8_t* data, const FrameInfo& f, const ScanHeader& sc, int16_t* const frame_coef[4], int* sync_passes)
+template <class Walk>
+bool emulate_sync_launch(uint32_t ns, int units, bool recording, Walk& walk, SubseqState* state, SyncScheduleCounts* counts)
+{
+    const bool paired = units == 2;
+    const uint32_t own = (uint32_t)units * kHuffOwn;
+    std::vector<uint64_t> from(ns, 0);
+    std::vector<uint64_t> end, start;
+    std::vector<int> tasks, next;
+    const auto assumed = [](uint32_t j) { return (uint64_t)j * kSubseqBits; };
+    for (uint32_t first = 0; first == 0 || first < ns; first += own) {
+        if (first >= ns) break;
+        const int n_rows = (int)std::min<uint32_t>(own + 1, ns - first + 1);
+        end.assign((size_t)n_rows, 0);
+        const auto decode = [&](int row, uint64_t at, bool record) {
+            const SubseqState p = unpack_state(at);
+            const uint32_t j = first - 1 + (uint32_t)row;
+            if (row > 0) from[j] = at & kSyncMask;
+            end[(size_t)row] = pack_state(walk(j, p.end_bit, p.zk & 255, p.zk >> 8, record));
+        };
+        for (int r = first ? 0 : (paired ? 2 : 1); r < n_rows; r += paired ? 2 : 1, counts->phase[0]++) decode(r, assumed(first - 1 + (uint32_t)r), false);
+        for (int r = 1; paired && r < n_rows; r += 2, counts->phase[1]++) decode(r, end[(size_t)r - 1], recording);
+        tasks.clear();
+        for (int r = paired ? 2 : 1; r < n_rows; r += paired ? 2 : 1)
+            if (recording || (end[(size_t)r - 1] & kSyncMask) != assumed(first - 1 + (uint32_t)r)) tasks.push_back(r);
+        for (int round = 1; !tasks.empty(); round++) {
+            if (round > n_rows + 2) return false;
+            if (round <= 2) counts->phase[round + 1] += tasks.size();
+            if (round == 3) counts->tail += tasks.size();
+            start.clear();
+            for (int r : tasks) start.push_back(end[(size_t)r - 1]);
+            next.clear();
+            for (size_t q = 0; q < tasks.size(); q++) {
+                const int r = tasks[q];
+                const uint64_t old = end[(size_t)r];
+                decode(r, start[q], recording);
+                if (((end[(size_t)r] ^ old) & kSyncMask) != 0 && r + 1 < n_rows) next.push_back(r + 1);
+            }
+            tasks.swap(next);
+        }
+        for (int r = 1; r < n_rows; r++) state[first - 1 + (uint32_t)r] = unpack_state(end[(size_t)r]);
+    }
+    for (uint32_t j = 1; j < ns; j++) {
+        const uint64_t at = pack_state(state[j - 1]);
+        if ((at & kSyncMask) == from[j]) continue;
+        const SubseqState p = unpack_state(at);
+        from[j] = at & kSyncMask;
+        state[j] = walk(j, p.end_bit, p.zk & 255, p.zk >> 8, recording);
+    }
+    return true;
+}
+
+int emulate_scan(const uint8_t* data, const FrameInfo& f, const ScanHeader& sc, int16_t* const frame_coef[4], int* sync_passes,
+                 SyncScheduleCounts* schedules)
 {
     std::vector<uint8_t> stream = device_scratch<uint8_t>(destuffed_capacity(sc));
     const size_t n = destuff_scan(data, sc, stream.data());
@@ -377,9 +429,10 @@
     std::vector<uint16_t> records = device_scratch<uint16_t>((size_t)ns * kRecShorts);
     bool forms_differ = false;
     uint16_t other[kRecShorts];
+    uint16_t* walk_records = records.data();
     auto walk = [&](uint32_t i, uint32_t begin, int z, int k, bool record) {
         const uint32_t limit = (i + 1) * kSubseqBits;
-        uint16_t* rec = &records[(size_t)i * kRecShorts];
+        uint16_t* rec = &walk_records[(size_t)i * kRecShorts];
         SubseqState st, sb;
         uint32_t mark = kRecInvalid;
         size_t named = 0;
@@ -396,7 +449,7 @@
             named = mark_valid(mark) ? 2 * (mark & (kRecFresh - 1)) : 0;
         }
         if (pack_state(st) != pack_state(sb) || memcmp(other, rec, named) != 0) forms_differ = true;
-        rec[kRecMark] = (uint16_t)mark;
+        if (record) rec[kRecMark] = (uint16_t)mark;
         return st;
     };
     for (uint32_t i = 0; i < ns; i++) cur[i] = walk(i, i * kSubseqBits, 0, 0, i == 0);
@@ -416,6 +469,26 @@
     }
     if (sync_passes) *sync_passes = passes;
     if (forms_differ) return 5;
+    for (int units = schedules ? 1 : 2; units <= 2; units++) {
+        std::vector<SubseqState> got = device_scratch<SubseqState>(ns);
+        std::vector<uint16_t> got_records = device_scratch<uint16_t>((size_t)ns * kRecShorts);
+        walk_records = got_records.data();
+        SyncScheduleCounts counts = {};
+        const bool ok = emulate_sync_launch(ns, units, !rst, walk, got.data(), &counts);
+        walk_records = records.data();
+        if (forms_differ || !ok) return 5;
+        for (uint32_t i = 0; i < ns; i++) {
+            const uint16_t *a = &records[(size_t)i * kRecShorts], *b = &got_records[(size_t)i * kRecShorts];
+            if (pack_state(got[i]) != pack_state(cur[i])) return 5;
+            if (rst) continue;
+            if (a[kRecMark] != b[kRecMark]) return 5;
+            if (mark_valid(a[kRecMark]) && memcmp(a, b, 2 * (a[kRecMark] & (kRecFresh - 1))) != 0) return 5;
+        }
+        if (schedules) {
+            for (int q = 0; q < 4; q++) schedules[units - 1].phase[q] += counts.phase[q];
+            schedules[units - 1].tail += counts.tail;
+        }
+    }
     if (!rst) {
         HostWindow win;
         win.env = &env;
@@ -501,14 +574,15 @@
 }
 }
 
-int emulate_gpu_entropy(const uint8_t* data, size_t size, const FrameInfo& f, int16_t* const coef[4], int* sync_passes)
+int emulate_gpu_entropy(const uint8_t* data, size_t size, const FrameInfo& f, int16_t* const coef[4], int* sync_passes, SyncScheduleCounts schedules[2])
 {
     (void)size;
     for (int c = 0; c < f.ncomp; c++) fill_device_scratch(coef[c], (size_t)f.comp[c].blocks_w * f.comp[c].blocks_h * 128);
     int passes = 0;
+    if (schedules) schedules[0] = schedules[1] = SyncScheduleCounts{};
     for (const ScanHeader& sc : f.scans) {
         int p = 0;
-        const int rc = emulate_scan(data, f, sc, coef, &p);
+        const int rc = emulate_scan(data, f, sc, coef, &p, schedules);
         passes = std::max(passes, p);
         if (rc != 0) return rc;
     }
diff --git a/nvimagecodec_amd/csrc/gpu_huffman_host.h b/nvimagecodec_amd/csrc/gpu_huffman_host.h
--- a/nvimagecodec_amd/csrc/gpu_huffman_host.h
+++ b/nvimagecodec_amd/csrc/gpu_huffman_host.h
@@ -27,6 +27,11 @@
 
 void fill_huff_image(const FrameInfo& f, const ScanHeader& sc, uint32_t stream_bytes, HuffImage* im);
 
-int emulate_gpu_entropy(const uint8_t* data, size_t size, const FrameInfo& f, int16_t* const coef[4], int* sync_passes);
+struct SyncScheduleCounts {
+    uint64_t phase[4];
+    uint64_t tail;
+};
+int emulate_gpu_entropy(const uint8_t* data, size_t size, const FrameInfo& f, int16_t* const coef[4], int* sync_passes,
+                        SyncScheduleCounts schedules[2] = nullptr);
 
 }
diff --git a/nvimagecodec_amd/csrc/hipjpeg_api.cpp b/nvimagecodec_amd/csrc/hipjpeg_api.cpp
--- a/nvimagecodec_amd/csrc/hipjpeg_api.cpp
+++ b/nvimagecodec_amd/csrc/hipjpeg_api.cpp
@@ -241,6 +241,32 @@
     });
 }
 
+hipjpegStatus_t hipjpegTestSyncScheduleCounts(const uint8_t* data, size_t length, uint64_t counts[10])
+{
+    return guarded([&]() -> hipjpegStatus_t {
+    if (!test_hooks_enabled() || !data || !counts) return HIPJPEG_STATUS_INVALID_ARGUMENT;
+    FrameInfo f;
+    ParseStatus ps = parse_jpeg(data, length, &f);
+    if (ps != kParseOk) return status_from_parse(ps);
+    if (gpu_progressive_eligible(f) || !gpu_entropy_eligible(f)) return HIPJPEG_STATUS_UNSUPPORTED;
+    std::vector<int16_t> coef(f.total_blocks() * 64);
+    int16_t* ptr[4] = {nullptr, nullptr, nullptr, nullptr};
+    size_t off = 0;
+    for (int c = 0; c < f.ncomp; c++) {
+        ptr[c] = coef.data() + off;
+        off += (size_t)f.comp[c].blocks_w * f.comp[c].blocks_h * 64;
+    }
+    SyncScheduleCounts schedules[2];
+    const int rc = emulate_gpu_entropy(data, length, f, ptr, nullptr, schedules);
+    for (int s = 0; s < 2; s++) {
+        for (int q = 0; q < 4; q++) counts[5 * s + q] = schedules[s].phase[q];
+        counts[5 * s + 4] = schedules[s].tail;
+    }
+    if (rc == 5) return HIPJPEG_STATUS_INTERNAL_ERROR;
+    return rc == 0 ? HIPJPEG_STATUS_SUCCESS : (rc == 2 ? HIPJPEG_STATUS_TRUNCATED : HIPJPEG_STATUS_CORRUPT);
+    });
+}
+
 hipjpegStatus_t hipjpegEntropyDecodeGpuIntervalAlgorithmHost(const uint8_t* data, size_t length, int16_t* coef, size_t coef_capacity_bytes,
                                                              uint64_t comp_offsets[4])
 {
diff --git a/nvimagecodec_amd/lowlevel.py b/nvimagecodec_amd/lowlevel.py
--- a/nvimagecodec_amd/lowlevel.py
+++ b/nvimagecodec_amd/lowlevel.py
@@ -98,6 +98,17 @@
         blk = buf[offs[c]: offs[c] + n * 64].reshape(info["blocks_h"][c], info["blocks_w"][c], 8, 8)
         coefs.append(np.ascontiguousarray(blk.transpose(0, 1, 3, 2)).reshape(info["blocks_h"][c], info["blocks_w"][c], 64))
     return coefs, passes.value
+
+
+def sync_schedule_counts(data):
+    a = _as_u8(data)
+    counts = (ctypes.c_uint64 * 10)()
+    fn = N.load().hipjpegTestSyncScheduleCounts
+    fn.argtypes = [ctypes.c_void_p, ctypes.c_size_t, ctypes.c_void_p]
+    st = fn(a.ctypes.data, a.size, ctypes.addressof(counts))
+    if st:
+        raise N.HipJpegError(st, "hipjpegTestSyncScheduleCounts")
+    return {name: {"phases": [int(v) for v in counts[5 * k:5 * k + 4]], "tail": int(counts[5 * k + 4])} for k, name in enumerate(("single", "paired"))}
 
 
 def entropy_decode_gpu_interval_algorithm_host(data):
```
